# MrSwordFish/rvel-mcmc

Measured on AMD Instinct MI355X. Metric: walker-logL evals/sec (2-planet, 100 obs, 4096 walkers); ESS/sec, higher is better.
Workload: dtype f64

## Files before the change

include/rvmcmc.h:

```cpp
#ifndef RVMCMC_H
#define RVMCMC_H

#include <stddef.h>
#include <stdint.h>

#ifdef __cplusplus
extern "C" {
#endif

#define RVM_ABI_VERSION 12

#define RVM_STATUS_OK 0
#define RVM_STATUS_PRIOR 1
#define RVM_STATUS_ENCOUNTER 2
#define RVM_STATUS_NONFINITE 3
#define RVM_STATUS_UNRESOLVED 4
#define RVM_STATUS_SKIPPED 5

#define RVM_MAX_PLANETS 4
#define RVM_MAX_LEVELS 6
#define RVM_MAX_EPOCHS_PER_DIRECTION 1700
#define RVM_SMALA_MAX_PARAMS 20
#define RVM_RESOLVE_MAX_LIMIT 12

typedef struct {
    int32_t n_planets;
    double dt;
    int32_t n_levels;
    double npoints_norm;
    int32_t level_mult[RVM_MAX_LEVELS];
    double period_hint;
    int32_t inclined;
    double resolve_tol;
    int32_t resolve_max;
} rvm_config;

typedef struct rvm_plan rvm_plan;

int rvm_plan_create(const rvm_config* cfg, const double* t, const double* rv, const double* sigma, int32_t n_obs,
                    int32_t max_walkers, rvm_plan** out);
void rvm_plan_destroy(rvm_plan* plan);
int rvm_plan_info(const rvm_plan* plan, int32_t* steps_fwd, int32_t* steps_bwd, int32_t* epochs_fwd,
                  int32_t* epochs_bwd);
#define RVM_EXT_MAX_BYTES (4ull << 30)
int rvm_plan_extension(const rvm_plan* plan, int32_t* ext_mult);
int rvm_plan_set_verify_eccentricity(rvm_plan* plan, double e);

int rvm_plan_set_certain_reject(rvm_plan* plan, int32_t on);

int rvm_plan_faults(rvm_plan* plan, int32_t reset, int64_t* handoff_timeouts, int64_t* nonfinite,
                    int64_t* unresolved, int64_t* refined, int64_t* truncated, void* stream);
#define RVM_N_COUNTERS 7
int rvm_plan_counters(rvm_plan* plan, int32_t reset, int64_t* out, int32_t n, void* stream);
int rvm_plan_hedge_stats(rvm_plan* plan, int32_t reset, int64_t* hedged, int64_t* replayed, int64_t* missed,
                         void* stream);
int rvm_plan_hedge_marks(rvm_plan* plan, int32_t reset, int64_t* marked, int64_t* gave_up, void* stream);
int rvm_plan_hedge_waits(rvm_plan* plan, int32_t reset, int64_t* waited, int64_t* late_hits, int64_t* gave_way,
                         void* stream);
int rvm_plan_time_kernels(rvm_plan* plan, int32_t max_launches);
int rvm_plan_kernel_times(rvm_plan* plan, float* logl_ms, float* refine_ms, int32_t max, int32_t* n_out);
int rvm_plan_set_handoff_timeout(rvm_plan* plan, double seconds);

int rvm_logl_batch(const rvm_plan* plan, int32_t n_walkers, const double* params, double hill_factor,
                   double* logl_out, int32_t* status_out, double* rv_out, void* stream);


int rvm_stretch_propose(int32_t n_params, int32_t n_s0, int64_t s0_begin, const double* x, int32_t n_s1,
                        const double* c, double a, uint64_t seed, uint64_t iteration, uint32_t half,
                        const double* draws, double* q_out, double* z_out, void* stream);
int rvm_stretch_accept(int32_t n_params, int32_t n_s0, int64_t s0_begin, double* x, double* lnp, const double* q,
                       const double* lnp_new, const double* z, uint64_t seed, uint64_t iteration, uint32_t half,
                       const double* draws, int32_t* accepted, void* stream);

#define RVM_MAX_PARAM_ROWS (7 * RVM_MAX_PLANETS)
typedef struct rvm_param_map {
    int32_t n_rows;
    int32_t src[RVM_MAX_PARAM_ROWS];
    double base[RVM_MAX_PARAM_ROWS];
} rvm_param_map;

int rvm_stretch_half_step(const rvm_plan* plan, const rvm_param_map* map, int32_t n_params, int32_t n_s0,
                          int64_t s0_begin, double* x, double* x_aos, double* lnp, int32_t n_s1, const double* c_aos,
                          double a, uint64_t seed, uint64_t iteration, uint32_t half, double hill_factor,
                          double* lnp_new_out, int32_t* status_out, int32_t* accepted, void* stream);

int rvm_stretch_iteration_begin(const rvm_plan* plan, const rvm_param_map* map, int32_t n_params, int32_t n_loc,
                                int64_t s0_begin, int64_t s1_begin, double* x0, double* lnp0, const double* x1,
                                const double* lnp1, int32_t n_half, const double* c0, const double* c1, double a,
                                uint64_t seed, uint64_t iteration, double hill_factor, double* lnp_spec,
                                int32_t* status_spec, int32_t* dec, int32_t* accepted0, void* stream);
int rvm_stretch_iteration_end(int32_t n_params, int32_t n_loc, int64_t s0_begin, int64_t s1_begin, const double* x0,
                              double* x0_aos, const int32_t* dec, const int32_t* dec_all, double* x1, double* x1_aos,
                              double* lnp1, int32_t n_half, const double* c0, const double* c1,
                              const double* lnp_spec, const int32_t* status_spec, double a, uint64_t seed,
                              uint64_t iteration, int32_t* accepted1, double* lnp_new_out, int32_t* status_new_out,
                              void* stream);

int rvm_pt_stretch_propose(int32_t n_params, int32_t n_temps, int32_t n_half, const double* x, const double* c,
                           double a, uint64_t seed, uint64_t iteration, uint32_t half, const double* draws,
                           double* q_out, double* z_out, void* stream);
int rvm_pt_stretch_accept(int32_t n_params, int32_t n_temps, int32_t n_half, const double* betas, double* x,
                          double* lnp, const double* q, const double* lnp_new, const double* z, uint64_t seed,
                          uint64_t iteration, uint32_t half, const double* draws, int32_t* accepted, void* stream);
int rvm_pt_swap(int32_t n_params, int32_t n_temps, int32_t n_half, const double* betas, double* x0, double* x1,
                double* lnp0, double* lnp1, uint64_t seed, uint64_t iteration, const double* draws,
                int32_t* swapped, void* stream);

int rvm_pt_ladder_update(int32_t n_temps, int32_t n_half, const int32_t* swapped, const double* lnp0,
                         const double* lnp1, double kappa, double* betas, int64_t* swap_totals_prev,
                         double* ratios_out, int64_t* n_refused, double* lnp_moments, void* workspace,
                         void* stream);

int rvm_mh_propose(int32_t n_params, int32_t n_chains, int64_t chain_begin, const double* x, const double* scales,
                   double step_size, uint64_t seed, uint64_t iteration, const double* draws, double* q_out,
                   void* stream);
int rvm_mh_accept(int32_t n_params, int32_t n_chains, int64_t chain_begin, double* x, double* lnp, const double* q,
                  const double* lnp_new, uint64_t seed, uint64_t iteration, const double* draws, int32_t* accepted,
                  void* stream);
int rvm_mh_step(const rvm_plan* plan, const rvm_param_map* map, int32_t n_params, int32_t n_chains,
                int64_t chain_begin, double* x, double* lnp, const double* scales, double step_size, uint64_t seed,
                uint64_t iteration, double hill_factor, double* lnp_new_out, int32_t* status_out, int32_t* accepted,
                void* stream);

int rvm_fd_params(int32_t n_params, int32_t n_chains, const double* x, double rel_step, const double* floor_,
                  double* out, void* stream);

typedef struct {
    double* lp;
    double* grad;
    double* mu;
    double* L;
    double* G;
    double* logdet;
    int32_t* ok;
} rvm_smala_cache;

int rvm_smala_derive(int32_t n_params, int32_t n_chains, int32_t n_obs, const double* x, double rel_step,
                     const double* floor_, const double* lp_stencil, const int32_t* status_stencil,
                     const double* rv_stencil, const double* inv_sigma2, double npoints_norm, double alpha,
                     double eps, const rvm_smala_cache* out, void* stream);
int rvm_smala_metric(int32_t n_params, int32_t n_chains, const double* x, const double* lp, const int32_t* status,
// ... 55 lines not shown
```

rvel-mcmc_amd/csrc/host_sanitize.cpp:

```cpp
#include <algorithm>
#include <cmath>
#include <cstdio>
#include <cstdlib>
#include <cstring>
#include <vector>

#include "rvm_plan_host.h"

static int fails = 0;
static void expect(bool ok, const char* what) {
    if (!ok) {
        std::fprintf(stderr, "FAIL %s\n", what);
        fails++;
    }
}

static double exact_weight(const int* m, int k0, int n, int k) {
    long long num = 1, den = 1;
    for (int j = k0; j < n; j++) {
        if (j == k) continue;
        num *= (long long)m[k] * m[k];
        den *= (long long)m[k] * m[k] - (long long)m[j] * m[j];
    }
    return (double)num / (double)den;
}

static bool close_rel(double a, double b, double rel) { return std::fabs(a - b) <= rel * std::fabs(b); }

static double ulp_of(double x) { return std::nextafter(std::fabs(x), INFINITY) - std::fabs(x); }

struct Range {
    size_t off, bytes;
    bool wide;
};
static void check_block(const std::vector<Range>& r, size_t block_bytes, const char* what) {
    size_t end = 0;
    for (const Range& x : r) {
        expect(x.off >= end, what);
        expect(!x.wide || x.off % 8 == 0, what);
        end = x.off + x.bytes;
    }
    expect(end <= block_bytes, what);
}

static const char* const kKnobNames[] = {
    "RVM_SKIP_VARIANTS", "RVM_LATE_SPO",   "RVM_NO_LEVEL_SPLIT", "RVM_REFINE_TEAMS", "RVM_EAGER_SPLIT",
    "RVM_NO_EXTENSION",  "RVM_REFINE_SPLIT", "RVM_TEAMS_HINT",   "RVM_EAGER",        "RVM_EAGER_PASSES",
    "RVM_HEDGE",         "RVM_HEDGE_GROUPS", "RVM_HEDGE_MARK",   "RVM_HEDGE_WAIT",
    "RVM_LS_F0"};

static rvm::PlanKnobs knobs_with(const char* name, const char* value) {
    setenv(name, value, 1);
    const rvm::PlanKnobs K = rvm::read_plan_knobs();
    unsetenv(name);
    return K;
}

static void check_plan_host(const rvm_config& cfg, const std::vector<double>& t, const std::vector<double>& rv,
                            const std::vector<double>& sg) {
    using namespace rvm;
    const int n_obs = (int)t.size();
    for (const char* name : kKnobNames) unsetenv(name);
    const PlanKnobs K = read_plan_knobs();
    expect(K.skip_variants == 1 && K.late_spo == 96.0 && !K.no_level_split && K.n_teams == RVM_TEAMS_DEFAULT &&
               K.eager_split == 1 && !K.no_extension && K.refine_split && K.teams_hint && K.eager &&
               K.eager_passes == 1 && K.hedge_groups == RVM_HEDGE_GROUPS_MAX && K.hedge_mark == 1 &&
               K.hedge_wait == 1,
           "knob defaults");
    expect(knobs_with("RVM_REFINE_TEAMS", "9").n_teams == RVM_TEAMS_MAX, "RVM_REFINE_TEAMS=9 clamps");
    expect(knobs_with("RVM_HEDGE", "0").hedge_groups == 0, "RVM_HEDGE=0");
    expect(knobs_with("RVM_HEDGE_GROUPS", "3").hedge_groups == 3, "RVM_HEDGE_GROUPS=3");
    expect(knobs_with("RVM_EAGER_PASSES", "2").eager_passes == 2, "RVM_EAGER_PASSES=2");
    expect(knobs_with("RVM_SKIP_VARIANTS", "0").skip_variants == 0, "RVM_SKIP_VARIANTS=0");
    expect(knobs_with("RVM_HEDGE_WAIT", "0").hedge_wait == 0 && knobs_with("RVM_HEDGE_WAIT", "1").hedge_wait == 1 &&
               knobs_with("RVM_HEDGE_WAIT", "2").hedge_wait == 2 && knobs_with("RVM_HEDGE_WAIT", "x").hedge_wait == 1,
           "RVM_HEDGE_WAIT");

    int mult[RVM_MAX_LEVELS] = {}, max_mult = 0;
    expect(check_plan_config(&cfg, t.data(), rv.data(), sg.data(), n_obs, 4096, mult, &max_mult) == nullptr,
           "config ok");
    expect(mult[0] == 4 && mult[1] == 5 && mult[2] == 6 && mult[3] == 7 && max_mult == 7, "explicit ladder");
    {
        rvm_config h = cfg;
        h.n_levels = 3;
        std::memset(h.level_mult, 0, sizeof(h.level_mult));
        int hm[RVM_MAX_LEVELS] = {}, hmax = 0;
        expect(check_plan_config(&h, t.data(), rv.data(), sg.data(), n_obs, 64, hm, &hmax) == nullptr && hm[0] == 1 &&
                   hm[1] == 2 && hm[2] == 3 && hmax == 3,
               "harmonic ladder");
    }

    HostDir dir[2];
    expect(build_schedule(&cfg, mult, max_mult, t.data(), rv.data(), sg.data(), n_obs, dir) == nullptr, "schedule ok");
    std::vector<int> seen(n_obs, 0);
    int n_dup = 0;
    for (int d = 0; d < 2; d++) {
        const HostDir& D = dir[d];
        const size_t n = D.idx.size();
        expect(D.seg_n.size() == n && D.seg_len.size() == n && D.orv.size() == n && D.os2.size() == n,
               "schedule sizes");
        long long sum = 0, pre0 = 0, pre1 = 0;
        double tprev = 0.0;
        for (size_t i = 0; i < n; i++) {
            const int o = D.idx[i];
            expect(o >= 0 && o < n_obs && (d == 0) == (t[o] >= 0.0), "obs_idx direction");
            if (o >= 0 && o < n_obs) seen[o]++;
            const double at = std::fabs(t[o]), len = (d == 0 ? 1.0 : -1.0) * (at - tprev);
            expect(at >= tprev, "|t| non-decreasing");
            if (at == tprev) {
                n_dup += i > 0;
                expect(D.seg_n[i] == 0 && D.seg_len[i] == 0.0, "duplicate epoch: empty segment");
            } else {
                expect(D.seg_n[i] >= 1 && std::fabs(D.seg_len[i]) <= cfg.dt * (1.0 + 1e-9), "segment step <= dt");
                expect(std::fabs(D.seg_n[i] * D.seg_len[i] - len) <= 4.0 * ulp_of(len), "segment steps x step = length");
            }
            tprev = at;
            if ((int)i < D.split0) pre0 += D.seg_n[i];
            if ((int)i < D.split1) pre1 += D.seg_n[i];
            sum += D.seg_n[i];
        }
        expect(sum == D.total_steps, "sum(seg_n) = n_steps");
        expect(D.split0 >= 0 && D.split0 <= (int)n && D.split1 >= 0 && D.split1 <= (int)n, "split range");
        expect(pre0 == D.pre0 && pre1 == D.pre1, "pre = steps before the split");
    }
    expect(std::all_of(seen.begin(), seen.end(), [](int c) { return c == 1; }), "obs_idx is a permutation");
    expect(n_dup == 1, "one duplicate epoch");

    const size_t nf = dir[0].idx.size(), nb = dir[1].idx.size();
    rvm_config ad = cfg;
    ad.resolve_tol = 5e-7;
    ad.resolve_max = 6;
    DevPlan P{};
    fill_plan_scalars(&ad, mult, n_obs, nf, nb, 256, K, &P);
    expect(P.ext_mult == 0 && plan_wants_extension(P, K), "extension wanted, not yet applied");
    fill_plan_extension(&P);
    const int m5[5] = {4, 5, 6, 7, 8};
    for (int k = 0; k < 4; k++) expect(close_rel(P.lw[k], exact_weight(m5, 0, 4, k), 1e-14), "lw");
    for (int k = 1; k < 4; k++) expect(close_rel(P.lw3[k], exact_weight(m5, 1, 4, k), 1e-14), "lw3");
    for (int k = 0; k < 5; k++) expect(close_rel(P.lw5[k], exact_weight(m5, 0, 5, k), 1e-14), "lw5");
    expect(P.lw3[0] == 0.0 && P.lw[4] == 0.0 && P.lw[5] == 0.0 && P.lw5[5] == 0.0, "unused weights are zero");

    expect(P.fin_level == 3, "fin_level");
    expect(P.ext_mult == 8 && P.mult[4] == 8 && P.inv_ext == 0.125 && P.inv_mult[4] == 0.125, "ext_mult");
    expect(P.rmax == 6 && P.rtol_dir == 2.5e-7 && P.cut == 1 && P.n_teams == RVM_TEAMS_DEFAULT, "adaptive scalars");
    expect(P.hedge_wait_ticks == hedge_wait_bound(P.spin_ticks) && P.hedge_wait_ticks < (P.spin_ticks << 1),
           "hedge_wait_ticks");
    for (unsigned long long sp : {1ull, 2ull, 3ull, 4ull, 1000ull, 200000000ull, 1ull << 40, 1ull << 62})
        expect(hedge_wait_bound(sp) < sp && hedge_wait_bound(sp) < (sp << 1), "hedge_wait_bound");
    for (int k = 0; k < 4; k++) {
        const double nh = 2.0 * M_PI * cfg.dt / (mult[k] * cfg.period_hint), zn = 2.0 * nh * nh;
        expect(P.nt[k] == (zn <= 0.1 ? 6 : (zn <= 0.3 ? 7 : 8)) && P.spec[k] == (zn <= 0.04 ? 1 : 0), "nt / spec");
        expect(P.inv_mult[k] == 1.0 / mult[k], "inv_mult");
    }
    expect(P.ext_nt == P.nt[3] && P.ext_spec == P.spec[3] && P.nt[4] == P.nt[3] && P.spec[4] == P.spec[3],
           "ext nt / spec");
    expect(P.late_mult == (int)std::ceil(96 * 0.65 / 5.2 - 1e-9) && P.late_mult == 12, "late_mult");
    expect(P.lc_ring >= 2 && P.lc_ring <= RVM_LC_RING, "lc_ring range");
    expect((size_t)(cfg.n_levels + 1) * 32 * 8 * P.lc_ring <= RVM_LC_RING_BYTES, "lc_ring bytes");
    {
        DevPlan Q{};
        fill_plan_scalars(&cfg, mult, n_obs, nf, nb, 256, K, &Q);
        expect(Q.rmax == 0 && !plan_wants_extension(Q, K) && Q.ext_mult == 0, "no extension without resolve_tol");
        ad.resolve_max = 0;
        fill_plan_scalars(&ad, mult, n_obs, nf, nb, 256, K, &Q);
        expect(!plan_wants_extension(Q, K) && Q.ext_mult == 0, "no extension with resolve_max 0");
        expect(!plan_wants_extension(P, knobs_with("RVM_NO_EXTENSION", "1")), "RVM_NO_EXTENSION=1");
        fill_plan_scalars(&cfg, mult, n_obs, nf, nb, 256, knobs_with("RVM_LATE_SPO", "0"), &Q);
        expect(Q.late_mult == 0, "RVM_LATE_SPO=0");
    }

    for (int32_t mw : {1, 64, 6144}) {
        const size_t w = (size_t)mw, em = std::max(nf, nb);
        const DmemLayout D = dmem_layout(nf, nb, mw);
        check_block({{D.seg_h1[0], 8 * nf, true}, {D.obs_rv[0], 8 * nf, true}, {D.obs_s2[0], 8 * nf, true},
                     {D.seg_h1[1], 8 * nb, true}, {D.obs_rv[1], 8 * nb, true}, {D.obs_s2[1], 8 * nb, true},
                     {D.slots, 8 * w, true}, {D.counters, 8 * RVM_N_COUNTERS, true}, {D.seg_n[0], 4 * nf, false},
                     {D.obs_idx[0], 4 * nf, false}, {D.seg_n[1], 4 * nb, false}, {D.obs_idx[1], 4 * nb, false}},
                    D.bytes, "dmem layout");
        const LvLayout V = lv_layout(nf, nb, mw);
        expect(V.emax == (int32_t)em, "lv emax");
        check_block({{V.rv, 8 * 2 * em * w, true}, {V.enc, 4 * 2 * w, false}}, V.bytes, "lvmem layout");
        for (int teams : {1, 2, 4}) {
            const size_t nt = (size_t)std::max(teams, 2), xg = (w + 15) / 16 + 1;
            const XLayout X = x_layout(nf, nb, mw, teams);
            check_block({{X.lvx, 16 * em * w, true}, {X.rvp, 16 * em * w, true},
                         {X.rvp2, 16 * em * w * (teams - 1), true}},
                        X.bytes, "xmem layout");
            const RqLayout R = rq_layout(mw, teams);
            expect(R.xgroups == (int32_t)xg, "rq xgroups");
            check_block({{R.x, xg * nt * 256 * 8, true}, {R.xf, xg * nt * 2 * 8, true},
                         {R.t, xg * (nt - 1) * 1024 * 8, true}, {R.tf, xg * nt * 8, true}, {R.tb, xg * 8, true},
                         {R.c, 16 * w, true},
                         {R.w, 12 * w, false}, {R.n, 16, false}, {R.gen, 8, true}, {R.mark, 4 * w, false},
                         {R.depth, 8 * (RVM_DEPTH_WINDOW + 1), true}},
                        R.bytes, "rqmem layout");
            expect(R.tb == R.tf + xg * nt * 8, "rq_tb right behind rq_tf");
            expect(R.gen == R.n + 32 && R.mark == R.n + 64 && R.mark % 64 == R.n % 64, "rq_n | gen_dev | rq_mark");
        }
        const HLayout H = h_layout((int32_t)em, mw);
        const size_t hs = RVM_HEDGE_STRIDE;
        check_block({{H.hrv, 16 * em * hs, true}, {H.hsum, 48 * hs, true}, {H.hslot, 16 * hs, true},
                     {H.htab, 8 * w, true}, {H.hw, 8 * RVM_HW_WORDS, true}},
                    H.bytes, "hmem layout");
        expect(RVM_HW_STATS + 5 <= RVM_HW_MARK && RVM_HW_MARK + 2 * RVM_HEDGE_GROUPS_MAX <= RVM_HW_WAIT &&
                   RVM_HW_WAIT + 3 <= RVM_HW_WORDS,
               "hw words");
        const ELayout E = e_layout((int32_t)em, mw);
        check_block({{E.rve, 32 * em * w, true}, {E.esum, 96 * w, true},
                     {E.eflag, 8 * (RVM_EFLAG_WORDS * (size_t)((RVM_EAGER_MAX + 15) / 16) + 8), true}},
                    E.bytes, "emem layout");
    }
}

int main() {
    expect(rvm_abi_version() == RVM_ABI_VERSION, "abi version");
    rvm_config cfg{};
    cfg.n_planets = 2;
    cfg.dt = 0.65;
    cfg.n_levels = 4;
    cfg.npoints_norm = 100.0;
    const int mult[4] = {4, 5, 6, 7};
    std::memcpy(cfg.level_mult, mult, sizeof(mult));
    cfg.period_hint = 5.2;
    std::vector<double> t, rv, sg;
    for (int i = 0; i < 101; i++) {
        t.push_back(i % 2 ? -0.6 * i : 0.55 * (100 - i));
        rv.push_back(1e-4 * std::sin(i));
        sg.push_back(1.5e-4);
    }
    t[7] = t[9];
    rvm_plan* plan = nullptr;
    const int rc = rvm_plan_create(&cfg, t.data(), rv.data(), sg.data(), (int)t.size(), 4096, &plan);
    expect(rc == 0 || (rc < 0 && plan == nullptr), "plan_create valid input");
    if (rc == 0) rvm_plan_destroy(plan);
    check_plan_host(cfg, t, rv, sg);
    rvm_config bad = cfg;
    bad.n_levels = 0;
    expect(rvm_plan_create(&bad, t.data(), rv.data(), sg.data(), (int)t.size(), 64, &plan) < 0, "n_levels 0");
    bad = cfg;
    bad.level_mult[1] = 4;
    expect(rvm_plan_create(&bad, t.data(), rv.data(), sg.data(), (int)t.size(), 64, &plan) < 0, "dup multipliers");
    bad = cfg;
    bad.dt = -1.0;
    expect(rvm_plan_create(&bad, t.data(), rv.data(), sg.data(), (int)t.size(), 64, &plan) < 0, "negative dt");
    std::vector<double> tn = t;
    tn[3] = NAN;
    expect(rvm_plan_create(&cfg, tn.data(), rv.data(), sg.data(), (int)t.size(), 64, &plan) < 0, "nan epoch");
    expect(std::strlen(rvm_last_error()) > 0, "last_error");
    expect(rvm_logl_batch(nullptr, 1, nullptr, 1.0, nullptr, nullptr, nullptr, nullptr) < 0, "logl null plan");
    int64_t mk = -1, gu = -1;
    expect(rvm_plan_hedge_marks(nullptr, 0, &mk, &gu, nullptr) < 0 && mk == -1 && gu == -1, "hedge_marks null plan");
    int64_t lh = -1;
    expect(rvm_plan_hedge_waits(nullptr, 0, &mk, &lh, &gu, nullptr) < 0 && mk == -1 && lh == -1 && gu == -1,
           "hedge_waits null plan");
    rvm_param_map pm{};
    expect(rvm_stretch_half_step(nullptr, &pm, 10, 1, 0, nullptr, nullptr, nullptr, 1, nullptr, 2.0, 0, 0, 0, 1.0,
                                 nullptr, nullptr, nullptr, nullptr) < 0,
           "half_step null plan");
    expect(rvm_stretch_propose(0, 1, 0, nullptr, 1, nullptr, 2.0, 0, 0, 0, nullptr, nullptr, nullptr, nullptr) < 0,
           "propose bad");
    double d1 = 0.5;
    int32_t i1 = 0;
    expect(rvm_pt_stretch_propose(10, 0, 1, &d1, &d1, 2.0, 0, 0, 0, nullptr, &d1, &d1, nullptr) < 0, "pt n_temps 0");
    expect(rvm_pt_stretch_propose(10, 2, 1, &d1, &d1, 1.0, 0, 0, 0, nullptr, &d1, &d1, nullptr) < 0, "pt a = 1");
    expect(rvm_pt_stretch_propose(10, 1 << 16, 1 << 16, &d1, &d1, 2.0, 0, 0, 0, nullptr, &d1, &d1, nullptr) < 0,
           "pt int32 overflow");
    expect(rvm_pt_stretch_accept(10, 2, 1, nullptr, &d1, &d1, &d1, &d1, &d1, 0, 0, 0, nullptr, &i1, nullptr) < 0,
           "pt null betas");
    expect(rvm_pt_stretch_accept(10, 2, 1, &d1, &d1, &d1, &d1, &d1, &d1, 0, 0, 2, nullptr, &i1, nullptr) < 0,
           "pt half 2");
    expect(rvm_pt_swap(10, 2, 0, &d1, &d1, &d1, &d1, &d1, 0, 0, nullptr, &i1, nullptr) < 0, "pt n_half 0");
    expect(rvm_pt_swap(10, 1 << 15, 1 << 15, &d1, &d1, &d1, &d1, &d1, 0, 0, nullptr, &i1, nullptr) < 0,
           "pt swap int32 overflow");
    expect(rvm_pt_swap(10, 1, 4, nullptr, nullptr, nullptr, nullptr, nullptr, 0, 0, nullptr, nullptr, nullptr) == 0,
           "pt swap of one temperature");
    int64_t l1 = 0;
    expect(rvm_pt_ladder_update(3, 1, &i1, &d1, &d1, -1.0, &d1, &l1, &d1, &l1, nullptr, &d1, nullptr) < 0,
           "pt ladder kappa < 0");
    expect(rvm_pt_ladder_update(3, 1, &i1, &d1, &d1, 0.5, &d1, &l1, &d1, &l1, nullptr, nullptr, nullptr) < 0,
           "pt ladder null workspace");
    expect(rvm_pt_ladder_update(1 << 16, 1 << 15, &i1, &d1, &d1, 0.5, &d1, &l1, &d1, &l1, nullptr, &d1, nullptr) < 0,
           "pt ladder int32 overflow");
    expect(rvm_pt_ladder_update(1, 4, nullptr, nullptr, nullptr, 0.5, nullptr, nullptr, nullptr, nullptr, nullptr,
                                nullptr, nullptr) == 0,
           "pt ladder of one temperature");
    expect(rvm_chain_record(2, 4, &d1, 16, 0, INT64_MAX, &d1, 8, 0, nullptr, nullptr, nullptr) < 0,
           "chain record stride overflow");
    expect(rvm_chain_record(2, 4, &d1, 16, 0, 1, &d1, INT64_MAX, INT64_MAX - 1, nullptr, nullptr, nullptr) < 0,
           "chain record dst_col0 overflow");
    expect(rvm_chain_record(2, 4, &d1, 16, 0, 1, &d1, 8, 0, &d1, nullptr, nullptr) < 0, "chain record lone lnp_src");
    expect(rvm_chain_moments(&d1, 2, 4, 5, 5, &d1, &d1, nullptr) < 0, "chain moments empty range");
    expect(rvm_chain_autocov(&d1, &d1, 2, 4, 0, 10, INT32_MAX, 1 << 30, &d1, &d1, nullptr) < 0,
           "chain autocov lag overflow");
    expect(rvm_chain_autocov(&d1, &d1, 65534, 4, 0, INT64_MAX, 0, 1 << 30, &d1, &d1, nullptr) < 0,
           "chain autocov n_params * n_lags");
    expect(rvm_chain_autocov_workspace_bytes(10, 200, 17) == (size_t)8 * 10 * 32, "chain autocov workspace");
    expect(rvm_chain_autocov_workspace_bytes(1, 65535 * 256, 1 << 30) == (size_t)8 * ((size_t)1 << 30) * 65535,
           "chain autocov workspace, largest");
    expect(rvm_chain_autocov_workspace_bytes(65534, 4, 1 << 30) == 0, "chain autocov workspace, refused");
    expect(rvm_mh_accept(0, 1, 0, nullptr, nullptr, nullptr, nullptr, 0, 0, nullptr, nullptr, nullptr) < 0, "mh bad");
    expect(rvm_fd_params(10, 1, nullptr, 1e-6, nullptr, nullptr, nullptr) < 0, "fd bad");
    const int32_t rows[2] = {0, 0};
    expect(rvm_logl_derivs(nullptr, 1, nullptr, 2, rows, 1.0, nullptr, nullptr, nullptr, nullptr, nullptr, nullptr) < 0,
           "derivs null plan");
    expect(rvm_logl_derivs_workspace_bytes(256, 10) == (size_t)256 * 55 * 2 * 36, "derivs workspace");
    rvm_smala_cache c{};
    expect(rvm_smala_metric(10, 1, nullptr, nullptr, nullptr, nullptr, nullptr, 1.0, 0.5, &c, nullptr) < 0, "metric bad");
    std::printf("host sanitize driver: %d failures\n", fails);
    return fails;
}
```

rvel-mcmc_amd/csrc/rvm_internal.h:

```cpp
#pragma once
#include <stdint.h>

#include "../../include/rvmcmc.h"

namespace rvm {

constexpr int RVM_LS_RING = 64;
constexpr int RVM_LC_RING = 16;
constexpr int RVM_LC_RING_BYTES = 24 * 1024;
constexpr int RVM_LDS_PER_CU = 160 * 1024;
constexpr int RVM_INIT_DOUBLES = 8 * 64;
constexpr double RVM_EXT_ACCEPT = 1.0;
constexpr double RVM_CUT_EST_FACTOR = 100.0;
constexpr double RVM_FLOOR_BOUND = 4.0;
constexpr double RVM_CUT_ECC_FACTOR = 0.6712;
constexpr double RVM_CUT_GUARD_K = 10.0;
constexpr int RVM_CX_MIN_WALKERS = 32;
constexpr int RVM_EAGER_MAX = 512;
constexpr int RVM_EAGER_MIN = 32;
constexpr int RVM_EFLAG_WORDS = 8;
constexpr int RVM_TEAMS_MAX = 4;
constexpr int RVM_TEAMS_DEFAULT = 4;
constexpr int RVM_DEPTH_WINDOW = 8;
constexpr int RVM_HEDGE_GROUPS_MAX = 8;
constexpr int RVM_HEDGE_STRIDE = 512;
constexpr int RVM_HEDGE_CAND = RVM_HEDGE_STRIDE + 64;
constexpr int RVM_HEDGE_MAX_W = 12288;
constexpr int RVM_HW_STATS = 2 + 2 * RVM_HEDGE_GROUPS_MAX;
constexpr int RVM_HW_MARK = RVM_HW_STATS + 3 + 3;
constexpr int RVM_HW_WAIT = RVM_HW_MARK + 2 * RVM_HEDGE_GROUPS_MAX;
constexpr int RVM_HW_WORDS = RVM_HW_WAIT + 3;

struct DirSched {
    int32_t n_epochs;
    int32_t n_steps;
    int32_t split0, pre0, split1, pre1;
    const int32_t* seg_n;
    const double* seg_h1;
    const double* obs_rv;
    const double* obs_s2;
    const int32_t* obs_idx;
};

struct DevPlan {
    int32_t n_planets;
    int32_t n_levels;
    int32_t mult[RVM_MAX_LEVELS];
    int32_t nt[RVM_MAX_LEVELS];
    int32_t spec[RVM_MAX_LEVELS];
    int32_t late_mult;
    int32_t lc_ring;
    double inv_mult[RVM_MAX_LEVELS];
    double lw[RVM_MAX_LEVELS];
    double lw3[RVM_MAX_LEVELS];
    double rtol_dir;
    int32_t rmax;
    int32_t fin_level;
    int32_t cut;
    int32_t ext_mult, ext_nt, ext_spec;
    double inv_ext;
    double lw5[RVM_MAX_LEVELS + 1];
    double* lvx;
    double* rvp;
    double e2_guard;
    double e2_cut;
    double cut_guard_k;
    int32_t lvx_emax, lvx_stride;
    int32_t* rq_n;
    int32_t* rq_w;
    double* rq_c;
    int32_t rq_cap;
    uint32_t hedge_wait_ticks;
    int32_t* rq_mark;
    int32_t skip_variants;
    unsigned long long* rq_x;
    unsigned long long* rq_xf;
    int32_t rq_xgroups;
    unsigned long long* rq_t;
    unsigned long long* rq_tf;
    double* rvp2;
    int32_t n_teams;
    unsigned long long* depth_w;
    double* rve;
    double* esum;
    unsigned long long* eflag;
    int32_t eager_max;
    int32_t eager_passes;
    int32_t eager_split;
    int32_t hedge_groups;
    int32_t hedge_mark;
    int32_t hedge_wait;
    double* hrv;
    double* hsum;
    unsigned long long* hslot;
    unsigned long long* htab;
    unsigned long long* hw;
    unsigned long long* gen_dev;
    unsigned long long* counters;
    unsigned long long spin_ticks;
    double npoints;
    int32_t n_obs;
    int32_t inclined;
    int32_t n_cu;
    double* lv_rv;
    int32_t* lv_enc;
    int32_t lv_emax, lv_stride;
    DirSched fwd, bwd;
};

struct StretchArgs {
    const double* c;
    double* x;
    double* x_aos;
    double* lnp;
    int32_t* accepted;
    int64_t s0_begin;
    uint64_t seed, iteration;
    double a;
    int32_t n1, dim;
    uint32_t half;
    int32_t xstride;
    int32_t n_spec;
    const double* c0;
    const double* x1;
    int64_t s1_begin;
    int32_t* dec;
    const double* lnp1;
    const double* mh_scale;
    double mh_step;
    const double* fd_x;
    const double* fd_floor;
    double fd_rel;
    int32_t fd_n;
    int32_t src[RVM_MAX_PARAM_ROWS];
    double base[RVM_MAX_PARAM_ROWS];
};

struct IterEndArgs {
    int32_t dim, n, n_half;
    int64_t s0_begin, s1_begin;
    const double* x0;
    double* x0_aos;
    const int32_t* dec_local;
    const int32_t* dec_all;
    double* x1;
    double* x1_aos;
    double* lnp1;
    const double* c0;
    const double* c1;
    const double* lnp_spec;
    const int32_t* st_spec;
    double a;
    uint64_t seed, iteration;
    int32_t* accepted1;
    double* lnp_new_out;
    int32_t* status_new_out;
};

struct PtLadderArgs {
    int32_t T, Wh;
    const int32_t* swapped;
    const double* lnp0;
    const double* lnp1;
    double kappa;
    double* betas;
    int64_t* totals_prev;
    double* ratios;
    int64_t* n_refused;
    double* moments;
    int64_t* ws_totals;
    double* ws_moments;
};

struct SmalaCache {
    double* lp;
    double* grad;
    double* mu;
    double* L;
    double* G;
    double* logdet;
    int32_t* ok;
};

}
```

rvel-mcmc_amd/csrc/rvm_logl.hip:

```cpp
#include <hip/hip_runtime.h>
#include <math.h>

#include <algorithm>

#pragma clang fp contract(on)

#include "rvm_launch.h"
#include "rvm_walker.h"

#ifndef RVM_MAIN_G5
#define RVM_MAIN_G5 0
#endif

namespace rvm {

#ifdef RVM_PROFILE
#define RVM_PROF_SLOTS 18
#define RVM_PROF_MAX_WAVES 4096
__device__ unsigned long long rvm_prof[RVM_PROF_MAX_WAVES * RVM_PROF_SLOTS];
#define PROF_T(v) const unsigned long long v = __builtin_readcyclecounter()
#define PROF_COUNT(var) (var)++
#else
#define PROF_T(v)
#define PROF_COUNT(var)
// ... 396 lines not shown
                __builtin_amdgcn_s_setprio(1);
            if (lvl == hl) {
                if (pl_idx == 0 && valid) {
                    unsigned long long bits = (unsigned long long)__double_as_longlong(v0);
                    if (bits == RVM_LV_EMPTY) bits = 0x7FF8000000000000ULL;
                    __hip_atomic_store(lv1p, bits, __ATOMIC_RELAXED, __HIP_MEMORY_SCOPE_AGENT);
                }
                lv1p += P.lv_stride;
            } else {
                if (E > RING && !wfault) {
                    int seen = -1;
                    for (;;) {
                        const int cp = __builtin_amdgcn_readfirstlane(
                            __hip_atomic_load(s_cprog + ul, __ATOMIC_ACQUIRE, __HIP_MEMORY_SCOPE_WORKGROUP));
                        if (e - cp < RING) break;
                        if (cp != seen) {
                            seen = cp;
                            clk.restart();
                        } else if (clk.expired(P.spin_ticks)) {
                            wfault = true;
                            break;
                        }
                        __builtin_amdgcn_s_sleep(4);
                    }
                }
                if (pl_idx == 0) ring[((ul * NK + ks) * RING + rslot) * WPB + slot] = v0;
                if (lane == 0) __hip_atomic_store(&s_lvp[ul][ks], e + 1, __ATOMIC_RELEASE, __HIP_MEMORY_SCOPE_WORKGROUP);
                rslot = rslot + 1 == RING ? 0 : rslot + 1;
            }
        } else {
            if (lc_pair) {
                rem -= ns * wcost;
                if (lane == 0) __hip_atomic_store(s_rem + wv, rem, __ATOMIC_RELAXED, __HIP_MEMORY_SCOPE_WORKGROUP);
                const int ro = __builtin_amdgcn_readfirstlane(rem_oth), rm = __builtin_amdgcn_readfirstlane(rem);
                if (__builtin_amdgcn_readfirstlane((int)(ro < rm)))
                    __builtin_amdgcn_s_setprio(2);
                else
                    __builtin_amdgcn_s_setprio(1);
            }
            if (lvl == 0) {
                while (!wfault && e - next_c >= RC) {
                    lc_wait(next_c);
                    if (!wfault) lc_combine(next_c++);
                }
            } else if (E > RC && !wfault && e >= RC) {
                int seen = -1;
                for (;;) {
                    const int cp = __builtin_amdgcn_readfirstlane(
                        __hip_atomic_load(&s_lcc[grp], __ATOMIC_ACQUIRE, __HIP_MEMORY_SCOPE_WORKGROUP));
                    if (e - cp < RC) break;
                    if (cp != seen) {
                        seen = cp;
                        clk.restart();
                    } else if (clk.expired(P.spin_ticks)) {
                        wfault = true;
                        break;
                    }
                    __builtin_amdgcn_s_sleep(4);
                }
            }
            if (pl_idx == 0) lring[((size_t)(e % RC) * (nl + 1) + lvl) * WPB + slot] = v0;
            if (lane == 0) __hip_atomic_store(&s_lcp[grp][lvl], e + 1, __ATOMIC_RELEASE, __HIP_MEMORY_SCOPE_WORKGROUP);
            if (lvl == 0 && !wfault) {
                const int mn = min(lc_min(), e + 1);
                while (next_c < mn) lc_combine(next_c++);
            }
        }
        n1 = n1_next;
        len = len_next;
#ifdef RVM_PROFILE
        PROF_T(tc);
        t_seg += tb - ta;
        t_epo += tc - tb;
#endif
    }
    if (!dec && lvl == 0) {
        while (!wfault && next_c < E_int) {
            lc_wait(next_c);
            if (!wfault) lc_combine(next_c++);
        }
    }
    const int encflag = (int)(((s.encm >> lane) & kick_enc_bits<NP>()) != 0) |
                        (status == RVM_STATUS_PRIOR ? 2 : 0) | (wfault ? RVM_ENC_FAULT : 0);
    auto finish = [&](const int wo, const double chi2w, const int enc, const bool open, const double lbw, auto&& row,
                      const double z, const double u3, const double lnp0) __attribute__((always_inline)) {
        const int st = dir_status(enc, open, chi2w);
        const unsigned long long mine =
            st != RVM_STATUS_OK ? slot_status(st)
                                : (unsigned long long)__double_as_longlong(open ? -lbw : chi2w);
        const unsigned long long old =
            __hip_atomic_exchange(slots + wo, mine, __ATOMIC_RELAXED, __HIP_MEMORY_SCOPE_AGENT);
        if (old == RVM_SLOT_EMPTY) return;
        __hip_atomic_store(slots + wo, RVM_SLOT_EMPTY, __ATOMIC_RELAXED, __HIP_MEMORY_SCOPE_AGENT);
        int st_o = RVM_STATUS_OK;
        bool open_o = false;
        double v_o = 0.0;
        if (slot_is_status(old)) {
            st_o = (int)(old & 0xFF);
        } else {
            v_o = __longlong_as_double((long long)old);
            open_o = signbit(v_o);
            v_o = fabs(v_o);
        }
        const double v_m = open ? lbw : chi2w;
        const int sf = d == 0 ? st : st_o, sb = d == 0 ? st_o : st;
        const bool of = d == 0 ? open : open_o, ob = d == 0 ? open_o : open;
        const double cf = d == 0 ? v_m : v_o, cb = d == 0 ? v_o : v_m;
        int stw = sf != RVM_STATUS_OK ? sf : sb;
        if (stw == RVM_STATUS_UNRESOLVED && (sf == RVM_STATUS_ENCOUNTER || sb == RVM_STATUS_ENCOUNTER))
            stw = RVM_STATUS_ENCOUNTER;
        const double lp0 = -((cb + cf) / P.npoints);
        if (stw == RVM_STATUS_OK && (of || ob)) {
            int dmode = 0;
            double dz, du, dl;
            if (P.ext_mult > 0 && P.cut) accept_inputs(sa, wo, dmode, dz, du, dl);
            if (dmode != 0 && isfinite(lp0) && !accepts_at(sa, dmode, dz, du, dl, lp0)) {
                __hip_atomic_fetch_add(P.counters + 4, (unsigned long long)((of ? 1 : 0) + (ob ? 1 : 0)),
                                       __ATOMIC_RELAXED, __HIP_MEMORY_SCOPE_AGENT);
            } else {
                const int li = of && ob ? 0 : (of ? 1 : 2);
                const int ix = __hip_atomic_fetch_add(P.rq_n + li, 1, __ATOMIC_RELAXED, __HIP_MEMORY_SCOPE_AGENT);
                if (ix < P.rq_cap) {
                    P.rq_w[(size_t)li * P.rq_cap + ix] = wo;
                    P.rq_mark[wo] = (int32_t)__hip_atomic_load(P.gen_dev, __ATOMIC_RELAXED, __HIP_MEMORY_SCOPE_AGENT);
                    P.rq_c[wo] = of ? 0.0 : cf;
                    P.rq_c[(size_t)P.rq_cap + wo] = ob ? 0.0 : cb;
                    return;
                }
                stw = RVM_STATUS_NONFINITE;
            }
        }
        if (stw == RVM_STATUS_OK && !isfinite(lp0)) stw = RVM_STATUS_NONFINITE;
        walker_out<R>(P, sa, wo, stw, stw == RVM_STATUS_OK ? lp0 : -INFINITY, logl_out, status_out, row, z, u3, lnp0);
    };
    auto finish_recompute = [&](const int w_in, const double chi2w, const int enc, const bool open, const double lbw) __attribute__((always_inline)) {
        if (stretch) {
            int wo = w_in, k2, wk2, j2, jp2;
            double z2, zp2;
            asm volatile("" : "+v"(wo));
            stretch_slot(sa, wo, k2, wk2, z2, j2, zp2, jp2);
            auto row = [&](int r) { return walker_param(true, params, W, wk2, sa, r, z2, j2, k2, zp2, jp2); };
            finish(wo, chi2w, enc, open, lbw, row, z2,
                   stretch_u3(sa.seed, (uint64_t)(sa.s0_begin + wo), sa.iteration, sa.half), k2 == 0 ? sa.lnp[wo] : 0.0);
        } else if (mh) {
            auto row = [&](int r) { return walker_param(true, params, W, w_in, sa, r, 0.0, 0, 0, 0.0, 0); };
            finish(w_in, chi2w, enc, open, lbw, row, 0.0, mh_u(sa.seed, (uint64_t)(sa.s0_begin + w_in), sa.iteration),
                   sa.lnp[w_in]);
        } else {
            auto row = [&](int) { return 0.0; };
            finish(w_in, chi2w, enc, open, lbw, row, 0.0, 0.0, 0.0);
        }
    };

    int dummy_redo = 0;
    auto extend_pass = [&](const int gr, const int dr, const uint64_t need_m, bool& need, double& chi2w, int& enc,
                           double& c5o, double& ddo) __attribute__((always_inline)) {
        const DirSched& SR = dr ? P.bwd : P.fwd;
        const int Er = SR.n_epochs;
        const double* r_dir = dec ? s_sched + (size_t)dr * 4 * emax2 : l_dir;
        const double* r_len = r_dir;
        const double* r_rv = r_dir + Er;
        const double* r_s2 = r_dir + 2 * Er;
        const int* r_n = reinterpret_cast<const int*>(r_dir + 3 * Er);
        const int* r_idx = r_n + Er;
        {
            const double* in = l_init + (size_t)gr * RVM_INIT_DOUBLES + lane;
            s.rx = in[0];
            s.ry = in[64];
            s.vx = in[128];
            s.vy = in[192];
            s.rz = in[256];
            s.vz = in[320];
            s.r = in[384];
            s.ir = in[448];
            s.encm = 0;
        }
        KickPrep<NP> kq{};
        if (Er > 0) kq = kick_prep<NP, L, D3>(s, 1.875);
        const int mx = P.ext_mult;
        const int ntx = P.ext_nt;
        const double ix = P.inv_ext;
        const int cs = lane & (WPB - 1);
        const bool cl = lane < WPB && ((need_m >> lane) & 1);
        const int wo = w0 + cs;
        const size_t xb = (size_t)dr * P.lvx_emax * P.lvx_stride + (cl ? wo : 0);
        const double* xs = P.lvx + xb;
        const double* xr = P.rvp + xb;
        double a5 = cl && Er > 0 ? xs[0] : 0.0, a4 = cl && Er > 0 ? xr[0] : 0.0;
        double c5 = 0.0, dd = 0.0;
        int x_off = 0, x_bo = 4;
        for (int e = 0; e < Er; e++) {
            const bool nx = cl && e + 1 < Er;
            const double b5 = nx ? xs[(size_t)(e + 1) * P.lvx_stride] : 0.0;
            const double b4 = nx ? xr[(size_t)(e + 1) * P.lvx_stride] : 0.0;
            const int ns = r_n[e] * mx;
            if (ns > 0) {
                const double h = r_len[e] * ix;
                if (P.ext_spec && ntx <= 6) {
                    if (x_off == 0) {
                        if (segment<6, true, D3, NP, L, RVM_MAIN_G5 != 0>(s, kq, h, ns, dummy_redo)) {
                            x_off = x_bo;
                            x_bo = x_bo < 64 ? 2 * x_bo : 64;
                        } else {
                            x_bo = 4;
                        }
                    } else {
                        segment<6, false, D3, NP, L, RVM_MAIN_G5 != 0>(s, kq, h, ns, dummy_redo);
                        x_off--;
                    }
                } else if (ntx <= 6)
                    segment<6, false, D3, NP, L, RVM_MAIN_G5 != 0>(s, kq, h, ns, dummy_redo);
                else if (ntx == 7)
                    segment<7, false, D3, NP, L, RVM_MAIN_G5 != 0>(s, kq, h, ns, dummy_redo);
                else
                    segment<8, false, D3, NP, L, RVM_MAIN_G5 != 0>(s, kq, h, ns, dummy_redo);
            }
            const double v = star_vx<NP, L>(s);
            const double vx = __shfl(v, cs * L);
            if (cl) {
                const double r = a4;
                const double r5 = a5 + P.lw5[nl] * vx;
                const double q = r5 - r_rv[e];
                c5 += (q * q) / r_s2[e];
                dd += fabs((r5 - r) * (q + (r - r_rv[e]))) / r_s2[e];
                if (rv_out != nullptr && wo < W) rv_out[(size_t)r_idx[e] * W + wo] = r5;
            }
            a5 = b5;
            a4 = b4;
        }
        const bool xenc = ((s.encm >> (cs * L)) & kick_enc_bits<NP>()) != 0;
        if (cl) {
            c5o = c5;
            ddo = dd;
// ... 286 lines not shown
                encc = (s_encl[ul][1][slot] | s_encl[ul][2][slot]) & 1;
                enc = s_encl[ul][0][slot] | ((s_encl[ul][1][slot] | s_encl[ul][2][slot]) & ~1);
            }
            {
                f1 = valid ? f1 : 0;
                if (ballot(f1 < 0) != 0 && !hung) {
                    do {
                        __builtin_amdgcn_s_sleep(2);
                        hung = clk.expired(P.spin_ticks);
                        f1 = valid ? __hip_atomic_load(e1p, __ATOMIC_RELAXED, __HIP_MEMORY_SCOPE_AGENT) : 0;
                    } while (ballot(f1 < 0) != 0 && !hung);
                }
                if (valid && pl_idx == 0) __hip_atomic_store(e1p, -1, __ATOMIC_RELAXED, __HIP_MEMORY_SCOPE_AGENT);
                const int f1p = f1 > 0 ? f1 : 0;
                if (P.rtol_dir < INFINITY) {
                    enc |= f1p & ~1;
                    encc |= f1p & 1;
                } else {
                    enc |= f1p;
                }
            }
            const bool cenc = encc != 0 && (enc & 1) == 0;
            if (hung) {
                chi2w = __builtin_nan("");
                enc |= RVM_ENC_FAULT;
                if (!dirty && lane == 0)
                    __hip_atomic_fetch_add(P.counters, 1ull, __ATOMIC_RELAXED, __HIP_MEMORY_SCOPE_AGENT);
            }
#ifdef RVM_PROFILE
            const unsigned long long rt_arr = __builtin_amdgcn_s_memrealtime();
#endif
            bool need = P.rtol_dir < INFINITY && valid && pl_idx == 0 && enc == 0 &&
                        (est / P.npoints > P.rtol_dir || !isfinite(chi2w) || !isfinite(est) ||
                         (P.ext_mult > 0 && e2w > P.e2_guard) || cenc);
            if (cenc && need && !lsx && P.ext_mult > 0)
                for (int e = 0; e < E; e++) P.rvp[(size_t)(d * P.lvx_emax + e) * P.lvx_stride + w] = __builtin_nan("");
            if (need && P.rmax == 0) {
                enc |= RVM_ENC_UNRESOLVED;
                need = false;
            }
            const bool need0 = need;
            const double chi2m = chi2w;
            if (lsx) {
                const uint64_t nx = ballot(need);
                if (lane == 0 && nx)
                    __hip_atomic_fetch_add(P.counters + 3, (unsigned long long)__builtin_popcountll(nx),
                                           __ATOMIC_RELAXED, __HIP_MEMORY_SCOPE_AGENT);
                if (need) {
                    if (s_encl[ul][3][slot] & 1) {
                        enc |= 1;
                        chi2w = c5x;
                        need = false;
                    } else if (!cenc && ddx <= RVM_EXT_ACCEPT * P.rtol_dir * P.npoints) {
                        chi2w = c5x;
                        need = false;
                    }
                }
            }
            if (!lsx && P.ext_mult > 0 && ballot(need) != 0) {
                if (valid && pl_idx == 0) {
                    s_fchi[ul][slot] = chi2w;
                    s_fenc[ul][slot] = enc | (need ? 16 : 0) | (cenc ? 32 : 0) | (e2w > P.e2_cut ? 64 : 0);
                    s_fx[0][ul][slot] = est;
                }
                __builtin_amdgcn_fence(__ATOMIC_RELEASE, "wavefront");
                __builtin_amdgcn_wave_barrier();
                const bool cl = lane < WPB && w0 + lane < W;
                double c2 = cl ? s_fchi[ul][lane] : 0.0;
                const int f = cl ? s_fenc[ul][lane] : 0;
                const double es = cl ? s_fx[0][ul][lane] : 0.0;
                const double cm = c2;
                int en = f & 15;
                bool nd = (f & 16) != 0;
                const bool cn = (f & 32) != 0;
                const uint64_t nm = ballot(nd);
                if (lane == 0)
                    __hip_atomic_fetch_add(P.counters + 3, (unsigned long long)__builtin_popcountll(nm),
                                           __ATOMIC_RELAXED, __HIP_MEMORY_SCOPE_AGENT);
                double xc5 = 0.0, xdd = 0.0;
                extend_pass(ul, d, nm, nd, c2, en, xc5, xdd);
                const double lb = cn ? 0.0 : direction_lb(nd, cm, es, (f & 16) != 0 && ((f & 64) == 0 || P.cut_guard_k > 0.0), xc5,
                                                                 (f & 64) != 0 ? P.cut_guard_k * xdd : xdd);
                if (cl) finish_recompute(w0 + lane, c2, en, nd, lb);
            } else if (valid && pl_idx == 0) {
                if (lsx && need) {
                    const double* rg = ring + (size_t)(ul * 4 + 2) * RING * WPB + slot;
                    for (int e = 0; e < E; e++)
                        P.rvp[(size_t)(d * P.lvx_emax + e) * P.lvx_stride + w] = cenc ? __builtin_nan("") : rg[(size_t)e * WPB];
                }
                finish_recompute(w, chi2w, enc, need,
                                 cenc ? 0.0 : direction_lb(need, chi2m, est, lsx && need0 && (e2w <= P.e2_cut || P.cut_guard_k > 0.0), c5x,
                                                          e2w <= P.e2_cut ? ddx : P.cut_guard_k * ddx));
            }
#ifdef RVM_PROFILE
            prof_dec(rt_arr, nl - 1);
#endif
        }
        return;
    }
#ifdef RVM_PROFILE
    PROF_T(t_end);
    const int gw = (blockIdx.y * gridDim.x + blockIdx.x) * (blockDim.x >> 6) + wv;
    if (lane == 0 && gw < RVM_PROF_MAX_WAVES) {
        unsigned long long* o = rvm_prof + (size_t)gw * RVM_PROF_SLOTS;
        o[0] = t_start;
        o[1] = t_pro;
        o[2] = t_seg;
        o[3] = t_epo;
        o[4] = t_end;
        o[5] = rt_start;
        o[6] = __builtin_amdgcn_s_memrealtime();
        o[7] = (unsigned long long)lvl | ((unsigned long long)blockIdx.y << 8) | ((unsigned long long)mult << 16);
        o[8] = (unsigned long long)redo;
        o[9] = (unsigned long long)E;
        o[10] = (unsigned long long)(unsigned)__builtin_amdgcn_s_getreg((31 << 11) | 4);
        o[14] = t_p1;
        o[15] = t_p2;
        o[16] = t_p3;
        o[17] = t_p4;
    }
#endif
}

template <int NPV, bool D3V, bool DECV>
static size_t lds_budget() {
    static size_t budget[64] = {};
    int dev = 0;
    if (hipGetDevice(&dev) != hipSuccess || dev < 0 || dev >= 64) {
        (void)hipGetLastError();
        return 32 * 1024;
    }
    if (budget[dev] == 0) {
        const void* f = reinterpret_cast<const void*>(&logl_kernel<NPV, D3V, DECV>);
        hipFuncAttributes fa{};
        size_t b = 32 * 1024;
        if (hipFuncGetAttributes(&fa, f) == hipSuccess && fa.sharedSizeBytes < (size_t)RVM_LDS_PER_CU) {
            const size_t lim = (size_t)RVM_LDS_PER_CU - fa.sharedSizeBytes;
            if (hipFuncSetAttribute(f, hipFuncAttributeMaxDynamicSharedMemorySize, (int)lim) == hipSuccess)
                b = lim;
            else if (fa.sharedSizeBytes < 64 * 1024)
                b = 64 * 1024 - fa.sharedSizeBytes;
        }
        (void)hipGetLastError();
        budget[dev] = b;
    }
    return budget[dev];
}

template <int NPV, bool D3V>
static hipError_t launch_logl_t(const DevPlan& P, int W, const double* params, double hill_factor,
                                unsigned long long* slots, double* logl, int32_t* status, double* rv_out,
                                const StretchArgs& sa, hipStream_t stream, int* dry_blocks) {
    const int lpw = LanesPerWalker<NPV>::value;
    const int wpb = 64 / lpw;
    const int groups = (W + wpb - 1) / wpb;
    static const bool pairs_env = [] {
        const char* e = getenv("RVM_CX_PAIRS");
        return !(e && e[0] == '0');
    }();
    const bool pairs = NPV == 3 && !D3V && pairs_env && P.ext_mult > 0 && rv_out == nullptr && P.n_cu > 0 &&
                       2 * groups > P.n_cu && groups <= P.n_cu && W >= RVM_CX_MIN_WALKERS;
    const int G = (!pairs && P.n_cu > 0 && 2 * groups > P.n_cu && 2 * P.n_levels * 64 <= 512) ? 2 : 1;
    dim3 grid((groups + G - 1) / G, 2);
    const bool cx = G == 1 && P.ext_mult > 0 && rv_out == nullptr && W >= RVM_CX_MIN_WALKERS;
    dim3 block(64 * (P.n_levels + (cx ? 1 : 0)) * G);
    const int emax = P.fwd.n_epochs > P.bwd.n_epochs ? P.fwd.n_epochs : P.bwd.n_epochs;
    const size_t rows = (size_t)(D3V ? 7 : 5) * NPV;
    const bool fused = sa.c != nullptr || sa.mh_scale != nullptr;
    const size_t init = P.rmax > 0 ? (size_t)RVM_INIT_DOUBLES * sizeof(double) : 0;
    const size_t lc_ring = (size_t)P.lc_ring * (P.n_levels + 1) * wpb * sizeof(double);
    size_t smem = (size_t)emax * 4 * sizeof(double) + (fused ? (rows + 3) * G * wpb * sizeof(double) : 0) + G * init +
                  G * lc_ring;
    int nA = 0, tB = 8, splitA = 0, lsx = 0;
    if (P.lv_rv != nullptr && W <= P.lv_stride && P.n_levels == 4 && P.n_cu > 0 && P.ext_mult > 0 &&
        rv_out == nullptr && G == 2 && emax <= RVM_LS_RING) {
        const int units = 2 * groups;
// ... 127 lines not shown
```

rvel-mcmc_amd/csrc/rvm_plan.hip:

```cpp
#include <algorithm>
#include <cmath>
#include <cstdlib>
#include <cstring>

#include "rvm_launch.h"
#include "rvm_plan.h"
#include "rvm_plan_host.h"

using rvm::fail;
using rvm::hip_fail;

namespace {

template <class T>
T* at(void* block, size_t offset) {
    return reinterpret_cast<T*>(reinterpret_cast<unsigned char*>(block) + offset);
}

template <class T>
const T* put(std::vector<unsigned char>& host, void* block, size_t offset, const std::vector<T>& v) {
    if (!v.empty()) std::memcpy(host.data() + offset, v.data(), v.size() * sizeof(T));
    return at<T>(block, offset);
}

// ... 15 lines not shown
    rvm::DirSched* S[2] = {&plan->dev.fwd, &plan->dev.bwd};
    for (int dd = 0; dd < 2; dd++) {
        const rvm::HostDir& D = dir[dd];
        S[dd]->n_epochs = (int32_t)D.idx.size();
        S[dd]->n_steps = plan->steps[dd] = (int32_t)D.total_steps;
        S[dd]->split0 = D.split0;
        S[dd]->pre0 = D.pre0;
        S[dd]->split1 = D.split1;
        S[dd]->pre1 = D.pre1;
        S[dd]->seg_h1 = put(host, plan->dmem, L.seg_h1[dd], D.seg_len);
        S[dd]->obs_rv = put(host, plan->dmem, L.obs_rv[dd], D.orv);
        S[dd]->obs_s2 = put(host, plan->dmem, L.obs_s2[dd], D.os2);
        S[dd]->seg_n = put(host, plan->dmem, L.seg_n[dd], D.seg_n);
        S[dd]->obs_idx = put(host, plan->dmem, L.obs_idx[dd], D.idx);
    }
    plan->slots = at<unsigned long long>(plan->dmem, L.slots);
    for (int32_t i = 0; i < max_walkers; i++)
        at<unsigned long long>(host.data(), L.slots)[i] = 0x7FF4DEADBEEF0001ULL;
    plan->dev.counters = at<unsigned long long>(plan->dmem, L.counters);
    plan->max_walkers = max_walkers;
    e = hipMemcpy(plan->dmem, host.data(), L.bytes, hipMemcpyHostToDevice);
    return e == hipSuccess ? 0 : hip_fail(e, "rvm_plan_create: hipMemcpy");
}

int device_cus() {
    int dev = 0, ncu = 0;
    if (hipGetDevice(&dev) != hipSuccess ||
        hipDeviceGetAttribute(&ncu, hipDeviceAttributeMultiprocessorCount, dev) != hipSuccess)
        ncu = 0;
    return ncu;
}

void alloc_level_split(rvm_plan* plan, size_t nf, size_t nb, const rvm::PlanKnobs& K) {
    rvm::DevPlan& P = plan->dev;
    if (!rvm::plan_wants_level_split(P, plan->max_walkers, K)) return;
    const rvm::LvLayout L = rvm::lv_layout(nf, nb, plan->max_walkers);
    if (!alloc_filled(&plan->lvmem, L.bytes, 0xFF)) return;
    P.lv_rv = at<double>(plan->lvmem, L.rv);
    P.lv_enc = at<int32_t>(plan->lvmem, L.enc);
    P.lv_emax = L.emax;
    P.lv_stride = plan->max_walkers;
    plan->lv_bytes = L.bytes;
}

void alloc_extension(rvm_plan* plan, size_t nf, size_t nb, const rvm::PlanKnobs& K) {
    rvm::DevPlan& P = plan->dev;
    if (!rvm::plan_wants_extension(P, K)) return;
    const rvm::XLayout L = rvm::x_layout(nf, nb, plan->max_walkers, K.n_teams);
    if (L.bytes > RVM_EXT_MAX_BYTES) return;
    if (hipMalloc(&plan->xmem, L.bytes) != hipSuccess) {
        plan->xmem = nullptr;
        (void)hipGetLastError();
        return;
    }
    rvm::fill_plan_extension(&P);
    P.lvx = at<double>(plan->xmem, L.lvx);
    P.rvp = at<double>(plan->xmem, L.rvp);
    P.rvp2 = K.n_teams >= 2 ? at<double>(plan->xmem, L.rvp2) : nullptr;
    P.lvx_emax = L.emax;
    P.lvx_stride = plan->max_walkers;
}

int alloc_work_lists(rvm_plan* plan, const rvm::PlanKnobs& K) {
    rvm::DevPlan& P = plan->dev;
    if (P.rmax <= 0) return 0;
    const rvm::RqLayout L = rvm::rq_layout(plan->max_walkers, K.n_teams);
    if (hipMalloc(&plan->rqmem, L.bytes) != hipSuccess || hipMemset(plan->rqmem, 0, L.bytes) != hipSuccess ||
        hipDeviceSynchronize() != hipSuccess) {
        (void)hipGetLastError();
        return fail(-3, "rvm_plan_create: hipMalloc of the refinement work lists failed");
    }
    P.rq_x = K.refine_split ? at<unsigned long long>(plan->rqmem, L.x) : nullptr;
    P.rq_xf = at<unsigned long long>(plan->rqmem, L.xf);
    P.rq_t = K.n_teams >= 2 ? at<unsigned long long>(plan->rqmem, L.t) : nullptr;
    P.rq_tf = at<unsigned long long>(plan->rqmem, L.tf);
    P.rq_c = at<double>(plan->rqmem, L.c);
    P.rq_w = at<int32_t>(plan->rqmem, L.w);
    P.rq_n = at<int32_t>(plan->rqmem, L.n);
    P.gen_dev = at<unsigned long long>(plan->rqmem, L.gen);
    P.rq_mark = at<int32_t>(plan->rqmem, L.mark);
    P.depth_w = K.teams_hint ? at<unsigned long long>(plan->rqmem, L.depth) : nullptr;
    P.rq_cap = plan->max_walkers;
    P.rq_xgroups = L.xgroups;
    const unsigned long long gen1 = 1;
    if (hipMemcpy(P.gen_dev, &gen1, sizeof(gen1), hipMemcpyHostToDevice) != hipSuccess) {
        (void)hipGetLastError();
        return fail(-3, "rvm_plan_create: initialising the launch generation failed");
    }
    return 0;
}

void side_drop(rvm_plan* plan) {
    (void)hipGetLastError();
    if (plan->ev_fork) (void)hipEventDestroy(plan->ev_fork);
    if (plan->ev_join) (void)hipEventDestroy(plan->ev_join);
    if (plan->side) (void)hipStreamDestroy(plan->side);
    plan->side = nullptr;
    plan->ev_fork = plan->ev_join = nullptr;
    plan->dev.hedge_groups = 0;
}

bool side_create(rvm_plan* plan) {
    if (hipStreamCreateWithFlags(&plan->side, hipStreamNonBlocking) == hipSuccess &&
        hipEventCreateWithFlags(&plan->ev_fork, hipEventDisableTiming) == hipSuccess &&
        hipEventCreateWithFlags(&plan->ev_join, hipEventDisableTiming) == hipSuccess)
        return true;
    side_drop(plan);
    return false;
}

void setup_side_features(rvm_plan* plan, const rvm::PlanKnobs& K) {
    rvm::DevPlan& P = plan->dev;
    const int32_t mw = plan->max_walkers;
    const bool refines = P.rmax >= 2 && P.rvp != nullptr && P.gen_dev != nullptr && P.n_levels <= 4 &&
                         mw >= rvm::RVM_EAGER_MIN;
    if (K.hedge_groups > 0 && refines && P.n_cu >= 4) {
        const rvm::HLayout L = rvm::h_layout(P.lvx_emax, mw);
        if (alloc_filled(&plan->hmem, L.bytes, 0)) {
            P.hrv = at<double>(plan->hmem, L.hrv);
            P.hsum = at<double>(plan->hmem, L.hsum);
            P.hslot = at<unsigned long long>(plan->hmem, L.hslot);
            P.htab = at<unsigned long long>(plan->hmem, L.htab);
            P.hw = at<unsigned long long>(plan->hmem, L.hw);
            P.hedge_groups = K.hedge_groups;
            P.hedge_mark = K.hedge_mark;
            P.hedge_wait = K.hedge_wait;
        }
    }
    if (!(refines && K.eager)) {
        if (P.hedge_groups > 0) (void)side_create(plan);
        return;
    }
    const rvm::ELayout L = rvm::e_layout(P.lvx_emax, P.lvx_stride);
    if (alloc_filled(&plan->emem, L.bytes, 0) && side_create(plan)) {
        P.rve = at<double>(plan->emem, L.rve);
        P.esum = at<double>(plan->emem, L.esum);
        P.eflag = at<unsigned long long>(plan->emem, L.eflag);
        P.eager_max = std::min<int>(mw, rvm::RVM_EAGER_MAX);
        P.eager_passes = K.eager_passes;
    } else {
        side_drop(plan);
        if (plan->emem) (void)hipFree(plan->emem);
        plan->emem = nullptr;
    }
}

int prepare_kernels(const rvm::DevPlan& P) {
    const hipError_t pe = rvm::prepare_logl(P);
    if (pe != hipSuccess)
        return fail(-1, pe == hipErrorInvalidConfiguration
                            ? "rvm_plan_create: the epoch schedule does not fit the likelihood kernel's LDS "
                              "(too many epochs in one direction)"
                            : "rvm_plan_create: n_planets has no kernel instantiation");
    if (rvm::prepare_refine(P) != hipSuccess)
        return fail(-1, "rvm_plan_create: the epoch schedule does not fit the refinement kernel's LDS "
                        "(too many epochs in one direction for the adaptive resolution)");
    return 0;
}

int read_hw_words(rvm_plan* plan, const char* who, int first, int n, int32_t reset, void* stream,
                  unsigned long long* h) {
    if (!plan) return fail(-1, std::string(who) + ": null plan");
    std::memset(h, 0, n * sizeof(*h));
    if (plan->dev.hw == nullptr) return 0;
    hipStream_t st = (hipStream_t)stream;
    unsigned long long* d = plan->dev.hw + first;
// ... 49 lines not shown
    if (plan->rqmem) (void)hipFree(plan->rqmem);
    if (plan->lvmem) (void)hipFree(plan->lvmem);
    if (plan->xmem) (void)hipFree(plan->xmem);
    if (plan->dmem) (void)hipFree(plan->dmem);
    delete plan;
}

int rvm_plan_set_certain_reject(rvm_plan* plan, int32_t on) {
    if (!plan) return fail(-1, "rvm_plan_set_certain_reject: null plan");
    plan->dev.cut = on ? 1 : 0;
    return 0;
}

int rvm_plan_set_verify_eccentricity(rvm_plan* plan, double e) {
    if (!plan) return fail(-1, "rvm_plan_set_verify_eccentricity: null plan");
    if (std::isnan(e) || e >= 1.0) return fail(-1, "rvm_plan_set_verify_eccentricity: e must be < 1 (<= 0: off)");
    plan->dev.e2_guard = e > 0.0 ? e * e : INFINITY;
    {
        const char* cf = getenv("RVM_CUT_FACTOR");
        const double ec = 1.0 - (1.0 - e) * (cf ? atof(cf) : rvm::RVM_CUT_ECC_FACTOR);
        const char* cg = getenv("RVM_CUT_GUARD");
        plan->dev.e2_cut = e > 0.0 && !(cg && atoi(cg) == 0) ? ec * ec : INFINITY;
        const char* ck = getenv("RVM_CUT_GUARD_K");
        plan->dev.cut_guard_k = ck ? atof(ck) : rvm::RVM_CUT_GUARD_K;
    }
    return 0;
}

int rvm_plan_extension(const rvm_plan* plan, int32_t* ext_mult) {
    if (!plan) return fail(-1, "rvm_plan_extension: null plan");
    if (ext_mult) *ext_mult = plan->dev.ext_mult;
    return 0;
}

int rvm_plan_counters(rvm_plan* plan, int32_t reset, int64_t* out, int32_t n, void* stream) {
    if (!plan) return fail(-1, "rvm_plan_counters: null plan");
    if (n < 0 || (n > 0 && !out)) return fail(-1, "rvm_plan_counters: bad output array");
    hipStream_t st = (hipStream_t)stream;
    unsigned long long h[RVM_N_COUNTERS] = {};
    hipError_t e = hipMemcpyAsync(h, plan->dev.counters, sizeof(h), hipMemcpyDeviceToHost, st);
    if (e == hipSuccess) e = hipStreamSynchronize(st);
    if (e != hipSuccess) return hip_fail(e, "rvm_plan_counters");
    for (int i = 0; i < n; i++) out[i] = i < RVM_N_COUNTERS ? (int64_t)h[i] : 0;
    if (reset) {
        if (plan->lvmem) e = hipMemsetAsync(plan->lvmem, 0xFF, plan->lv_bytes, st);
        if (e == hipSuccess) e = hipMemsetAsync(plan->dev.counters, 0, sizeof(h), st);
        if (e == hipSuccess) e = hipStreamSynchronize(st);
        if (e != hipSuccess) return hip_fail(e, "rvm_plan_counters: reset");
    }
    return 0;
}

int rvm_plan_hedge_stats(rvm_plan* plan, int32_t reset, int64_t* hedged, int64_t* replayed, int64_t* missed,
                         void* stream) {
    unsigned long long h[3];
    const int rc = read_hw_words(plan, "rvm_plan_hedge_stats", rvm::RVM_HW_STATS, 3, reset, stream, h);
    if (rc != 0) return rc;
    if (hedged) *hedged = (int64_t)h[0];
    if (replayed) *replayed = (int64_t)h[1];
    if (missed) *missed = (int64_t)h[2];
    return 0;
}

int rvm_plan_hedge_marks(rvm_plan* plan, int32_t reset, int64_t* marked, int64_t* gave_up, void* stream) {
    unsigned long long h[2];
    const int rc = read_hw_words(plan, "rvm_plan_hedge_marks", rvm::RVM_HW_STATS + 3, 2, reset, stream, h);
    if (rc != 0) return rc;
    if (marked) *marked = (int64_t)h[0];
    if (gave_up) *gave_up = (int64_t)h[1];
    return 0;
}

int rvm_plan_hedge_waits(rvm_plan* plan, int32_t reset, int64_t* waited, int64_t* late_hits, int64_t* gave_way,
                         void* stream) {
    unsigned long long h[3];
    const int rc = read_hw_words(plan, "rvm_plan_hedge_waits", rvm::RVM_HW_WAIT, 3, reset, stream, h);
    if (rc != 0) return rc;
    if (waited) *waited = (int64_t)h[0];
    if (late_hits) *late_hits = (int64_t)h[1];
    if (gave_way) *gave_way = (int64_t)h[2];
    return 0;
}

int rvm_plan_faults(rvm_plan* plan, int32_t reset, int64_t* handoff_timeouts, int64_t* nonfinite,
                    int64_t* unresolved, int64_t* refined, int64_t* truncated, void* stream) {
    if (!plan) return fail(-1, "rvm_plan_faults: null plan");
    int64_t c[RVM_N_COUNTERS] = {};
    const int rc = rvm_plan_counters(plan, reset, c, RVM_N_COUNTERS, stream);
    if (rc != 0) return rc;
    if (handoff_timeouts) *handoff_timeouts = c[0];
    if (nonfinite) *nonfinite = c[1];
    if (unresolved) *unresolved = c[2];
    if (refined) *refined = c[3];
    if (truncated) *truncated = c[4];
    return 0;
}

int rvm_plan_time_kernels(rvm_plan* plan, int32_t max_launches) {
    if (!plan) return fail(-1, "rvm_plan_time_kernels: null plan");
    if (max_launches < 0 || max_launches > 4096) return fail(-1, "rvm_plan_time_kernels: max_launches out of range");
    while ((int32_t)plan->tev.size() < 3 * max_launches) {
        hipEvent_t ev;
        const hipError_t e = hipEventCreate(&ev);
        if (e != hipSuccess) return hip_fail(e, "rvm_plan_time_kernels: hipEventCreate");
        plan->tev.push_back(ev);
    }
    plan->tcap = max_launches;
    plan->tn = 0;
    return 0;
}

int rvm_plan_kernel_times(rvm_plan* plan, float* logl_ms, float* refine_ms, int32_t max, int32_t* n_out) {
    if (!plan || max < 0) return fail(-1, "rvm_plan_kernel_times: bad arguments");
    const int n = std::min(plan->tn, max);
    for (int i = 0; i < n; i++) {
        hipError_t e = hipEventSynchronize(plan->tev[3 * i + 2]);
        float a = 0.0f, b = 0.0f;
        if (e == hipSuccess) e = hipEventElapsedTime(&a, plan->tev[3 * i], plan->tev[3 * i + 1]);
        if (e == hipSuccess) e = hipEventElapsedTime(&b, plan->tev[3 * i + 1], plan->tev[3 * i + 2]);
        if (e != hipSuccess) return hip_fail(e, "rvm_plan_kernel_times");
        if (logl_ms) logl_ms[i] = a;
        if (refine_ms) refine_ms[i] = b;
    }
    if (n_out) *n_out = n;
    plan->tn = 0;
    plan->tcap = 0;
    return 0;
}

int rvm_plan_set_handoff_timeout(rvm_plan* plan, double seconds) {
    if (!plan) return fail(-1, "rvm_plan_set_handoff_timeout: null plan");
    if (!(seconds > 0.0) || !(seconds < 1e9)) return fail(-1, "rvm_plan_set_handoff_timeout: seconds out of range");
    const double ticks = seconds * 1e8;
    plan->dev.spin_ticks = ticks < 1.0 ? 1ull : (unsigned long long)ticks;
    plan->dev.hedge_wait_ticks = rvm::hedge_wait_bound(plan->dev.spin_ticks);
    return 0;
}

int rvm_plan_info(const rvm_plan* plan, int32_t* sf, int32_t* sb, int32_t* ef, int32_t* eb) {
    if (!plan) return fail(-1, "rvm_plan_info: null plan");
    if (sf) *sf = plan->steps[0];
    if (sb) *sb = plan->steps[1];
    if (ef) *ef = plan->dev.fwd.n_epochs;
    if (eb) *eb = plan->dev.bwd.n_epochs;
    return 0;
}

}
```

rvel-mcmc_amd/csrc/rvm_plan_host.cpp:

```cpp
#include "rvm_plan_host.h"

#include <algorithm>
#include <cmath>
#include <cstdlib>

#ifndef RVM_EAGER_DEFAULT
#define RVM_EAGER_DEFAULT true
#endif
#ifndef RVM_EAGER_PASSES_DEFAULT
#define RVM_EAGER_PASSES_DEFAULT 1
#endif

namespace rvm {

static bool starts(const char* s, char c) { return s && s[0] == c; }

PlanKnobs read_plan_knobs() {
    PlanKnobs K;
    K.skip_variants = starts(getenv("RVM_SKIP_VARIANTS"), '0') ? 0 : 1;
    const char* ls = getenv("RVM_LATE_SPO");
    K.late_spo = ls ? atof(ls) : 96.0;
    K.no_level_split = false;
#ifdef RVM_PROFILE
    K.no_level_split = starts(getenv("RVM_NO_LEVEL_SPLIT"), '1');
#endif
    K.n_teams = RVM_TEAMS_DEFAULT;
    if (const char* tp = getenv("RVM_REFINE_TEAMS")) K.n_teams = std::max(1, std::min(atoi(tp), RVM_TEAMS_MAX));
    K.eager_split = starts(getenv("RVM_EAGER_SPLIT"), '0') ? 0 : 1;
    K.no_extension = starts(getenv("RVM_NO_EXTENSION"), '1');
    K.refine_split = !starts(getenv("RVM_REFINE_SPLIT"), '0');
    K.teams_hint = !starts(getenv("RVM_TEAMS_HINT"), '0');
    const char* eg = getenv("RVM_EAGER");
    K.eager = eg ? eg[0] == '1' : RVM_EAGER_DEFAULT;
    const char* ep = getenv("RVM_EAGER_PASSES");
    K.eager_passes = starts(ep, '1') ? 1 : (starts(ep, '2') ? 2 : RVM_EAGER_PASSES_DEFAULT);
    K.hedge_groups = starts(getenv("RVM_HEDGE"), '0') ? 0 : RVM_HEDGE_GROUPS_MAX;
    if (const char* hn = getenv("RVM_HEDGE_GROUPS"))
        K.hedge_groups = std::min(K.hedge_groups, std::max(0, std::min(atoi(hn), (int)RVM_HEDGE_GROUPS_MAX)));
    K.hedge_mark = starts(getenv("RVM_HEDGE_MARK"), '0') ? 0 : 1;
    const char* hwt = getenv("RVM_HEDGE_WAIT");
    K.hedge_wait = starts(hwt, '0') ? 0 : (starts(hwt, '2') ? 2 : 1);
    return K;
}

const char* check_plan_config(const rvm_config* cfg, const double* t, const double* rv, const double* sigma,
                              int32_t n_obs, int32_t max_walkers, int mult[RVM_MAX_LEVELS], int* max_mult) {
    if (cfg->n_planets < 1 || cfg->n_planets > RVM_MAX_PLANETS) return "rvm_plan_create: n_planets out of range";
    if (cfg->n_levels < 1 || cfg->n_levels > RVM_MAX_LEVELS) return "rvm_plan_create: n_levels out of range";
    if (!(cfg->dt > 0.0) || !std::isfinite(cfg->dt)) return "rvm_plan_create: dt must be > 0";
    if (n_obs < 0 || max_walkers < 1) return "rvm_plan_create: bad sizes";
    if (!(cfg->npoints_norm != 0.0)) return "rvm_plan_create: npoints_norm must be nonzero";
    bool harmonic = true;
    for (int k = 0; k < cfg->n_levels; k++) harmonic = harmonic && cfg->level_mult[k] == 0;
    *max_mult = 1;
    for (int k = 0; k < cfg->n_levels; k++) {
        mult[k] = harmonic ? k + 1 : cfg->level_mult[k];
        if (mult[k] < 1 || mult[k] > 64) return "rvm_plan_create: level_mult out of range (1..64)";
        for (int j = 0; j < k; j++)
            if (mult[j] == mult[k]) return "rvm_plan_create: level_mult entries must be distinct";
        *max_mult = std::max(*max_mult, mult[k]);
    }
    if (!(cfg->period_hint >= 0.0) || !std::isfinite(cfg->period_hint))
        return "rvm_plan_create: period_hint must be >= 0";
    if (std::isnan(cfg->resolve_tol) || cfg->resolve_max < 0 || cfg->resolve_max > RVM_RESOLVE_MAX_LIMIT)
        return "rvm_plan_create: resolve_tol must be a number and resolve_max in 0..12";
    for (int i = 0; i < n_obs; i++)
        if (!std::isfinite(t[i]) || !std::isfinite(rv[i]) || !std::isfinite(sigma[i]))
            return "rvm_plan_create: non-finite observation";
    return nullptr;
}

static void split_point(const HostDir& D, double frac, int32_t* split, int32_t* pre) {
    const double target = frac * (double)D.total_steps;
    long long cum = 0, best_cum = 0;
    int best = 0;
    double best_d = target;
    for (size_t i = 0; i < D.seg_n.size(); i++) {
        cum += D.seg_n[i];
        const double dist = std::fabs((double)cum - target);
        if (dist < best_d) {
            best_d = dist;
            best = (int)i + 1;
            best_cum = cum;
        }
    }
    *split = best;
    *pre = (int32_t)best_cum;
}

const char* build_schedule(const rvm_config* cfg, const int* mult, int max_mult, const double* t, const double* rv,
                           const double* sigma, int32_t n_obs, HostDir dir[2]) {
    const int rmax = cfg->resolve_tol > 0.0 ? cfg->resolve_max : 0;
    double f0 = 0.5;
    if (cfg->n_levels == 4) f0 = (double)(mult[3] + mult[0] - mult[2]) / (2.0 * mult[0]) + 0.11;
#ifdef RVM_PROFILE
    if (const char* ef = getenv("RVM_LS_F0")) f0 = atof(ef);
#endif
    f0 = std::min(1.0, std::max(0.0, f0));
    for (int dd = 0; dd < 2; dd++) {
        HostDir& D = dir[dd];
        for (int i = 0; i < n_obs; i++)
            if ((dd == 0) == (t[i] >= 0.0)) D.idx.push_back(i);
        std::stable_sort(D.idx.begin(), D.idx.end(), [&](int a, int b) { return std::fabs(t[a]) < std::fabs(t[b]); });
        const double sign = dd == 0 ? 1.0 : -1.0;
        double tprev = 0.0;
        for (int i : D.idx) {
            const double at = std::fabs(t[i]);
            const double len = at - tprev;
            tprev = at;
            int n = len > 0.0 ? (int)std::ceil(len / cfg->dt - 1e-9) : 0;
            if (len > 0.0 && n < 1) n = 1;
            D.seg_n.push_back(n);
            D.seg_len.push_back(n > 0 ? sign * len / n : 0.0);
            D.orv.push_back(rv[i]);
            D.os2.push_back(sigma[i] * sigma[i]);
            D.total_steps += n;
        }
        if ((D.total_steps * (long long)max_mult) << rmax > (1LL << 30))
            return "rvm_plan_create: dt too small for the epoch span";
        if (D.idx.size() > (size_t)RVM_MAX_EPOCHS_PER_DIRECTION)
            return "rvm_plan_create: too many epochs in one direction (the schedule is staged in LDS)";
        split_point(D, f0, &D.split0, &D.pre0);
        split_point(D, 0.5, &D.split1, &D.pre1);
    }
// ... 76 lines not shown
void fill_plan_extension(DevPlan* Pp) {
    DevPlan& P = *Pp;
    const int nl = P.n_levels, fin = P.fin_level;
    int m5[RVM_MAX_LEVELS + 1];
    for (int k = 0; k < nl; k++) m5[k] = P.mult[k];
    m5[nl] = P.mult[fin] + 1;
    lagrange_at_zero(m5, 0, nl + 1, P.lw5);
    P.ext_mult = m5[nl];
    P.ext_nt = P.nt[fin];
    P.ext_spec = P.spec[fin];
    P.inv_ext = 1.0 / m5[nl];
    P.mult[nl] = P.ext_mult;
    P.nt[nl] = P.ext_nt;
    P.spec[nl] = P.ext_spec;
    P.inv_mult[nl] = P.inv_ext;
}

bool plan_wants_level_split(const DevPlan& P, int32_t max_walkers, const PlanKnobs& K) {
    const int wpb = walkers_per_group(P.n_planets);
    const int64_t groups = ((int64_t)max_walkers + wpb - 1) / wpb;
    bool inc = P.n_levels == 4 && !K.no_level_split;
    for (int k = 1; inc && k < 4; k++) inc = P.mult[k] > P.mult[k - 1];
    return inc && P.n_cu > 0 && 2 * groups > P.n_cu;
}

static size_t take(size_t& end, size_t bytes) {
    end += bytes;
    return end - bytes;
}
static size_t epochs_max(size_t nf, size_t nb) { return std::max<size_t>(std::max(nf, nb), 1); }

DmemLayout dmem_layout(size_t nf, size_t nb, int32_t max_walkers) {
    DmemLayout L{};
    const size_t n[2] = {nf, nb};
    for (int d = 0; d < 2; d++) {
        L.seg_h1[d] = take(L.bytes, n[d] * sizeof(double));
        L.obs_rv[d] = take(L.bytes, n[d] * sizeof(double));
        L.obs_s2[d] = take(L.bytes, n[d] * sizeof(double));
    }
    L.slots = take(L.bytes, (size_t)max_walkers * sizeof(unsigned long long));
    L.counters = take(L.bytes, RVM_N_COUNTERS * sizeof(unsigned long long));
    for (int d = 0; d < 2; d++) {
        L.seg_n[d] = take(L.bytes, n[d] * sizeof(int32_t));
        L.obs_idx[d] = take(L.bytes, n[d] * sizeof(int32_t));
    }
    L.bytes += 64;
    return L;
}

LvLayout lv_layout(size_t nf, size_t nb, int32_t max_walkers) {
    LvLayout L{};
    L.emax = (int32_t)epochs_max(nf, nb);
    L.rv = take(L.bytes, (size_t)(2 * (int64_t)L.emax * max_walkers) * sizeof(double));
    L.enc = take(L.bytes, (size_t)(2 * (int64_t)max_walkers) * sizeof(int32_t));
    return L;
}

XLayout x_layout(size_t nf, size_t nb, int32_t max_walkers, int n_teams) {
    XLayout L{};
    L.emax = (int32_t)epochs_max(nf, nb);
    const size_t bl = 2 * (size_t)L.emax * (size_t)max_walkers * sizeof(double);
    L.lvx = take(L.bytes, bl);
    L.rvp = take(L.bytes, bl);
    L.rvp2 = take(L.bytes, ((size_t)n_teams - 1) * bl);
    return L;
}

RqLayout rq_layout(int32_t max_walkers, int n_teams) {
    RqLayout L{};
    const size_t xg = (size_t)(((int64_t)max_walkers + 15) / 16 + 1), nt = (size_t)std::max(n_teams, 2);
    const size_t u64 = sizeof(unsigned long long);
    L.xgroups = (int32_t)xg;
    L.x = take(L.bytes, xg * nt * 2 * 2 * 64 * u64);
    L.xf = take(L.bytes, xg * nt * 2 * u64);
    L.t = take(L.bytes, xg * (nt - 1) * 16 * 64 * u64);
    L.tf = take(L.bytes, xg * nt * u64);
    L.tb = take(L.bytes, xg * u64);
    L.c = take(L.bytes, 2 * (size_t)max_walkers * sizeof(double));
    L.w = take(L.bytes, (3 * (size_t)max_walkers * sizeof(int32_t) + 7) & ~(size_t)7);
    L.n = take(L.bytes, 64);
    L.gen = L.n + 32;
    L.mark = take(L.bytes, ((size_t)max_walkers * sizeof(int32_t) + 63) & ~(size_t)63);
    L.depth = take(L.bytes, (RVM_DEPTH_WINDOW + 1) * u64);
    return L;
}

HLayout h_layout(int32_t lvx_emax, int32_t max_walkers) {
    HLayout L{};
    const size_t hs = RVM_HEDGE_STRIDE, w = sizeof(double);
    L.hrv = take(L.bytes, 2 * (size_t)lvx_emax * hs * w);
    L.hsum = take(L.bytes, 6 * hs * w);
    L.hslot = take(L.bytes, 2 * hs * w);
    L.htab = take(L.bytes, (size_t)max_walkers * w);
    L.hw = take(L.bytes, RVM_HW_WORDS * w);
    return L;
}

ELayout e_layout(int32_t lvx_emax, int32_t lvx_stride) {
    ELayout L{};
    const size_t plane = (size_t)lvx_emax * lvx_stride;
    L.rve = take(L.bytes, 4 * plane * sizeof(double));
    L.esum = take(L.bytes, 12 * (size_t)lvx_stride * sizeof(double));
    L.eflag = take(L.bytes, (RVM_EFLAG_WORDS * (size_t)((RVM_EAGER_MAX + 15) / 16) + 8) * sizeof(double));
    return L;
}

}
```

rvel-mcmc_amd/csrc/rvm_plan_host.h:

```cpp
#pragma once
#include <cstddef>
#include <vector>

#include "rvm_internal.h"

namespace rvm {

struct PlanKnobs {
    int32_t skip_variants;
    double late_spo;
    bool no_level_split;
    int32_t n_teams;
    int32_t eager_split;
    bool no_extension;
    bool refine_split;
    bool teams_hint;
    bool eager;
    int32_t eager_passes;
    int32_t hedge_groups;
    int32_t hedge_mark;
    int32_t hedge_wait;
};
PlanKnobs read_plan_knobs();

const char* check_plan_config(const rvm_config* cfg, const double* t, const double* rv, const double* sigma,
                              int32_t n_obs, int32_t max_walkers, int mult[RVM_MAX_LEVELS], int* max_mult);

struct HostDir {
    std::vector<int32_t> idx, seg_n;
    std::vector<double> seg_len, orv, os2;
    long long total_steps = 0;
    int32_t split0 = 0, pre0 = 0, split1 = 0, pre1 = 0;
};
const char* build_schedule(const rvm_config* cfg, const int* mult, int max_mult, const double* t, const double* rv,
                           const double* sigma, int32_t n_obs, HostDir dir[2]);

void lagrange_at_zero(const int* m, int k0, int n, double* w);

inline int walkers_per_group(int n_planets) { return n_planets == 1 ? 64 : (n_planets == 2 ? 32 : 16); }

void fill_plan_scalars(const rvm_config* cfg, const int* mult, int32_t n_obs, size_t nf, size_t nb, int n_cu,
                       const PlanKnobs& K, DevPlan* P);
uint32_t hedge_wait_bound(unsigned long long spin_ticks);
bool plan_wants_extension(const DevPlan& P, const PlanKnobs& K);
void fill_plan_extension(DevPlan* P);
bool plan_wants_level_split(const DevPlan& P, int32_t max_walkers, const PlanKnobs& K);

struct DmemLayout {
    size_t seg_h1[2], obs_rv[2], obs_s2[2], slots, counters, seg_n[2], obs_idx[2], bytes;
};
DmemLayout dmem_layout(size_t nf, size_t nb, int32_t max_walkers);
struct LvLayout {
    size_t rv, enc, bytes;
    int32_t emax;
};
LvLayout lv_layout(size_t nf, size_t nb, int32_t max_walkers);
struct XLayout {
    size_t lvx, rvp, rvp2, bytes;
    int32_t emax;
};
XLayout x_layout(size_t nf, size_t nb, int32_t max_walkers, int n_teams);
struct RqLayout {
    size_t x, xf, t, tf, tb, c, w, n, gen, mark, depth, bytes;
    int32_t xgroups;
};
RqLayout rq_layout(int32_t max_walkers, int n_teams);
struct HLayout {
    size_t hrv, hsum, hslot, htab, hw, bytes;
};
HLayout h_layout(int32_t lvx_emax, int32_t max_walkers);
struct ELayout {
    size_t rve, esum, eflag, bytes;
};
ELayout e_layout(int32_t lvx_emax, int32_t lvx_stride);

}
```

rvel-mcmc_amd/csrc/rvm_refine_impl.h:

```cpp
#pragma once
#include <hip/hip_runtime.h>
#include <math.h>

#pragma clang fp contract(on)

#include "rvm_walker.h"

#ifndef RVM_REFINE_GUESS
#define RVM_REFINE_GUESS 0
#endif
#ifndef RVM_REFINE_RELAXED_COUNT
#define RVM_REFINE_RELAXED_COUNT 0
#endif

namespace rvm {

#ifdef RVM_PROFILE
#define RVM_RPROF_SLOTS 24
#define RVM_RPROF_MAX_WAVES 4096
static __device__ unsigned long long rvm_rprof[RVM_RPROF_MAX_WAVES * RVM_RPROF_SLOTS];
#define RPROF_T(v) const unsigned long long v = __builtin_readcyclecounter()
#define RPROF_RT(v) const unsigned long long v = __builtin_amdgcn_s_memrealtime()
#else
#define RPROF_T(v)
// ... 2 lines not shown

__device__ __forceinline__ bool claim_item(gu64* w, unsigned long long gen, unsigned long long code) {
    unsigned long long v = __hip_atomic_load(w, __ATOMIC_RELAXED, __HIP_MEMORY_SCOPE_AGENT);
    for (;;) {
        if ((v >> 8) == gen) return false;
        unsigned long long expect = v;
        if (__hip_atomic_compare_exchange_strong(w, &expect, (gen << 8) | code, __ATOMIC_RELAXED, __ATOMIC_RELAXED,
                                                 __HIP_MEMORY_SCOPE_AGENT))
            return true;
        v = expect;
    }
}

__device__ __forceinline__ void hedge_mark_unneeded(const int32_t* rq_w, const int rq_cap,
                                                    const unsigned long long* htab, unsigned long long* hw_,
                                                    const int n0, const int n1, const int n2,
                                                    const unsigned long long gen, const int hedge, const int wpb) {
    const int lane = threadIdx.x & 63;
    unsigned need = 0;
    for (int l2 = 0; l2 < 3; l2++) {
        int n = l2 == 0 ? n0 : (l2 == 1 ? n1 : n2);
        n = n < rq_cap ? n : rq_cap;
        for (int i = lane; i < n; i += 64) {
            const int wl = rq_w[(size_t)l2 * rq_cap + i];
            if (wl < 0 || wl >= rq_cap) continue;
            const unsigned long long tb = __hip_atomic_load((gu64*)htab + wl, __ATOMIC_RELAXED, __HIP_MEMORY_SCOPE_AGENT);
            const int hg = (int)(tb & 0xFFFF) / wpb;
            if ((tb >> 16) != gen || hg >= RVM_HEDGE_GROUPS_MAX) continue;
            if (l2 != 2) need |= 1u << (2 * hg);
            if (l2 != 1) need |= 1u << (2 * hg + 1);
        }
    }
    for (int d = 32; d >= 1; d >>= 1) need |= (unsigned)__shfl_xor((int)need, d, 64);
    gu64* hw = (gu64*)hw_;
    const bool mark = lane < hedge && lane < 2 * RVM_HEDGE_GROUPS_MAX && !((need >> lane) & 1u);
    if (mark) __hip_atomic_store(hw + RVM_HW_MARK + lane, (gen << 8) | 1ull, __ATOMIC_RELAXED, __HIP_MEMORY_SCOPE_AGENT);
    const unsigned long long nm = __builtin_popcountll(ballot(mark));
    if (lane == 0 && nm)
        __hip_atomic_fetch_add(hw + RVM_HW_STATS + 3, nm, __ATOMIC_RELAXED, __HIP_MEMORY_SCOPE_AGENT);
}

__device__ __forceinline__ int hedge_wait_poll(const DevPlan& P, const unsigned long long gen, const int wme,
                                               const bool o0, const bool o1, const int wpb, const gu64* tbw,
                                               const gu64* tdone) {
    const unsigned long long done = (gen << 8) | 2ull, stop = (gen << 8) | 3ull;
    auto state = [&](const int dd, const bool want) -> int {
        if (!want) return 0;
        const unsigned long long tb = __hip_atomic_load((gu64*)P.htab + wme, __ATOMIC_RELAXED, __HIP_MEMORY_SCOPE_AGENT);
        const int ix = (int)(tb & 0xFFFF);
        if ((tb >> 16) != gen || ix >= RVM_HEDGE_STRIDE || ix / wpb >= RVM_HEDGE_GROUPS_MAX) return 2;
        if (__hip_atomic_load((gu64*)P.hslot + (size_t)dd * RVM_HEDGE_STRIDE + ix, __ATOMIC_RELAXED,
                              __HIP_MEMORY_SCOPE_AGENT) != ((gen << 16) | (unsigned long long)wme))
            return 2;
        const unsigned long long w =
            __hip_atomic_load((gu64*)P.hw + 2 + 2 * (ix / wpb) + dd, __ATOMIC_RELAXED, __HIP_MEMORY_SCOPE_AGENT);
        return w == done ? 0 : (w == stop ? 2 : 1);
    };
    SpinClock clk;
    clk.restart();
    for (bool first = true;; first = false) {
        const int s0 = state(0, o0), s1 = state(1, o1);
        if (ballot(s0 == 2 || s1 == 2) != 0) return first ? -1 : 0;
        if (ballot(s0 == 1 || s1 == 1) == 0) return 1;
        const bool give = __hip_atomic_load(tbw, __ATOMIC_RELAXED, __HIP_MEMORY_SCOPE_AGENT) == ((gen << 8) | 1ull) ||
                          __hip_atomic_load(tdone, __ATOMIC_RELAXED, __HIP_MEMORY_SCOPE_AGENT) == done ||
                          clk.expired(P.hedge_wait_ticks);
        if (__builtin_amdgcn_readfirstlane((int)give)) return 0;
        __builtin_amdgcn_s_sleep(2);
    }
}

__device__ __forceinline__ unsigned long long pass_ticks(const DevPlan& P, int rf) {
    const unsigned long long t = P.spin_ticks << (rf < RVM_RESOLVE_MAX_LIMIT ? rf : RVM_RESOLVE_MAX_LIMIT);
    constexpr unsigned long long cap = 6000000000ull;
    return t < cap ? t : (P.spin_ticks > cap ? P.spin_ticks : cap);
}

struct DirState {
    int open;
    double chi, lb, pest, best, bchi;
};

constexpr int RVM_REFINE_HM = 5;
template <int NP, bool D3, int NW>
__global__ __launch_bounds__((NW == RVM_REFINE_HM ? 4 : NW) * 64) void refine_kernel(
    const DevPlan P, const int W, const double* __restrict__ params, const double hill_factor,
    double* __restrict__ rv_out, double* __restrict__ logl_out, int32_t* __restrict__ status_out, const StretchArgs sa,
    const int eager, const int hedge) {
    constexpr bool HM = NW == RVM_REFINE_HM;
    constexpr int L = LanesPerWalker<NP>::value;
    constexpr int WPB = 64 / L;
    constexpr int PR = D3 ? 7 : 5;
    constexpr int R = PR * NP;
    const int wv = threadIdx.x >> 6;
    const int lane = threadIdx.x & 63;
    const int slot = lane / L;
    const int pl_idx = lane % L;
    const int nl = P.n_levels;
    RPROF_T(pt_entry);
    RPROF_RT(prt_entry);
#ifdef RVM_PROFILE
    unsigned long long p_seg = 0, p_epo = 0, p_steps = 0, p_wait = 0, p_pass = 0;
    unsigned long long p_look = 0, p_info = 0, p_need = 0, p_barr = 0;
    int p_lvl = -1;
#endif

    __shared__ int s_n[3];
    __shared__ unsigned long long s_gen;
    __shared__ int s_depth;
    if (threadIdx.x == 0) {
        for (int i = 0; i < 3; i++) s_n[i] = __hip_atomic_load(P.rq_n + i, __ATOMIC_RELAXED, __HIP_MEMORY_SCOPE_AGENT);
        const unsigned long long g0 = __hip_atomic_load(P.gen_dev, __ATOMIC_RELAXED, __HIP_MEMORY_SCOPE_AGENT);
        s_gen = g0;
        int d = P.depth_w != nullptr ? 0 : RVM_TEAMS_MAX;
        if (P.depth_w != nullptr) {
            unsigned long long v[RVM_DEPTH_WINDOW];
#pragma unroll
            for (int i = 0; i < RVM_DEPTH_WINDOW; i++)
                v[i] = __hip_atomic_load(P.depth_w + (g0 + 1 + i) % (RVM_DEPTH_WINDOW + 1), __ATOMIC_RELAXED,
                                         __HIP_MEMORY_SCOPE_AGENT);
#pragma unroll
            for (int i = 0; i < RVM_DEPTH_WINDOW; i++)
                if ((v[i] >> 8) < g0 && (v[i] >> 8) + RVM_DEPTH_WINDOW >= g0 && (int)(v[i] & 0xFF) > d)
                    d = (int)(v[i] & 0xFF);
        }
        s_depth = d;
#if RVM_REFINE_RELAXED_COUNT
        asm volatile("s_waitcnt vmcnt(0)" ::: "memory");
        const int done = __hip_atomic_fetch_add(P.rq_n + 3, 1, __ATOMIC_RELAXED, __HIP_MEMORY_SCOPE_AGENT);
#else
        const int done = __hip_atomic_fetch_add(P.rq_n + 3, 1, __ATOMIC_ACQ_REL, __HIP_MEMORY_SCOPE_AGENT);
#endif
        if (done == (int)gridDim.x - 1) {
            for (int i = 0; i < 4; i++) __hip_atomic_store(P.rq_n + i, 0, __ATOMIC_RELAXED, __HIP_MEMORY_SCOPE_AGENT);
            if (!eager && !hedge) __hip_atomic_store(P.gen_dev, g0 + 1, __ATOMIC_RELAXED, __HIP_MEMORY_SCOPE_AGENT);
        }
    }
    __syncthreads();
    RPROF_T(pt_lists);
    const unsigned long long gen = s_gen;
    const int nq[3] = {s_n[0], s_n[1], s_n[2]};
    const int depth_hint = s_depth;
    const int gq0 = (nq[0] + WPB - 1) / WPB, gq1 = (nq[1] + WPB - 1) / WPB, gq2 = (nq[2] + WPB - 1) / WPB;
    const int ng = gq0 + gq1 + gq2;
    const int ntask_split = 2 * gq0 + gq1 + gq2;
    const int gfit = hedge && P.n_cu - hedge < (int)gridDim.x ? P.n_cu - hedge : (int)gridDim.x;
    auto leave = [&]() {
        if (hedge && threadIdx.x == 0) {
            gu64* hw = (gu64*)P.hw;
            if (__hip_atomic_fetch_add(hw + 1, 1ull, __ATOMIC_RELAXED, __HIP_MEMORY_SCOPE_AGENT) + 1 == gridDim.x) {
                __hip_atomic_store(hw + 1, 0ull, __ATOMIC_RELAXED, __HIP_MEMORY_SCOPE_AGENT);
                __hip_atomic_store(hw, (gen << 8) | 1ull, __ATOMIC_RELAXED, __HIP_MEMORY_SCOPE_AGENT);
            }
        }
    };
    const bool split = !eager && P.rq_x != nullptr && gq0 <= P.rq_xgroups && ((int)gridDim.x & 1) == 0 &&
                       ntask_split <= gfit;
    int nteam = 0;
    if (split && P.rq_t != nullptr && P.rvp != nullptr && P.rvp2 != nullptr && rv_out == nullptr &&
        ng <= P.rq_xgroups) {
        nteam = P.n_teams < P.rmax ? P.n_teams : P.rmax;
        if (nteam > (depth_hint > 2 ? depth_hint : 2)) nteam = depth_hint > 2 ? depth_hint : 2;
        while (nteam >= 2 && nteam * ntask_split > gfit) nteam--;
    }
    const bool team = nteam >= 2;
    const int ntask_team = nteam * ntask_split;
    const int ngw = (W + WPB - 1) / WPB;
    const bool esplit = eager && P.eager_split && P.rq_x != nullptr && ngw <= P.rq_xgroups &&
                        ((int)gridDim.x & 1) == 0 && 2 * ngw <= (int)gridDim.x;
    const int ntask = eager ? (esplit ? 2 * ngw : ngw) : (team ? ntask_team : (split ? ntask_split : ng));
    if ((int)blockIdx.x >= ntask) {
        if constexpr (HM) {
            if (hedge && P.hedge_mark && blockIdx.x == gridDim.x - 1 && wv == 0)
                hedge_mark_unneeded(P.rq_w, P.rq_cap, P.htab, P.hw, nq[0], nq[1], nq[2], gen, hedge, WPB);
        }
        leave();
        return;
    }

    extern __shared__ double s_sched[];
    __shared__ double s_rv[2][2][RVM_MAX_LEVELS][64];
    __shared__ int s_enc[2][RVM_MAX_LEVELS][64];
    __shared__ double s_init[8][64];
    __shared__ double s_chi[2][64], s_lb[2][64];
    __shared__ double s_pest[2][64], s_best[2][64], s_bchi[2][64];
    __shared__ int s_open[2][64];
    __shared__ int s_live[64];
    __shared__ int s_stw[64];
    __shared__ double s_lpw[64];
    __shared__ double s_acc[3][64];
    __shared__ int s_dmode[64];
    __shared__ unsigned long long s_mask[2];
    __shared__ int s_xfault;
    __shared__ double s_tc2[2][64], s_te2[2][64];
    __shared__ int s_ter[2][64];
    __shared__ int s_cancel[2];
    __shared__ int s_eitems[64], s_eli[64], s_eany;
    __shared__ int s_emask;
    __shared__ int s_hix[2][64];
    __shared__ int s_skip[64];
    const int emax = P.fwd.n_epochs > P.bwd.n_epochs ? P.fwd.n_epochs : P.bwd.n_epochs;
    for (int dd = 0; dd < 2; dd++) {
        const DirSched& SD = dd ? P.bwd : P.fwd;
        double* b = s_sched + (size_t)dd * 4 * emax;
        const int ED = SD.n_epochs;
        int* bn = reinterpret_cast<int*>(b + 3 * ED);
        for (int i = threadIdx.x; i < ED; i += blockDim.x) {
            b[i] = SD.seg_h1[i];
            b[ED + i] = SD.obs_rv[i];
            b[2 * ED + i] = SD.obs_s2[i];
            bn[i] = SD.seg_n[i];
            bn[ED + i] = SD.obs_idx[i];
        }
    }
    RPROF_T(pt_sched);
    const bool stretch = sa.c != nullptr;
    const bool mh = sa.mh_scale != nullptr;
    const bool mapped = stretch || mh || sa.fd_x != nullptr;

    for (int t = blockIdx.x; t < ntask; t += gridDim.x) {
        int g = t, own = -1, tm = 0;
        if (team) {
            if (t < 2 * nteam * gq0) {
                g = t / (2 * nteam);
                const int r = t - g * 2 * nteam;
                own = r & 1;
                tm = r >> 1;
            } else {
                const int u = t - 2 * nteam * gq0;
                g = gq0 + u / nteam;
                tm = u - (u / nteam) * nteam;
            }
        } else if (esplit) {
            g = t >> 1;
            own = t & 1;
        } else if (split) {
            if (t < 2 * gq0) {
                g = t >> 1;
                own = t & 1;
            } else {
                g = t - gq0;
            }
        }
        int li = g < gq0 ? 0 : (g < gq0 + gq1 ? 1 : 2);
        const int base = (li == 0 ? g : (li == 1 ? g - gq0 : g - gq0 - gq1)) * WPB;
        int cnt = nq[li] - base < WPB ? nq[li] - base : WPB;
        const int* items = P.rq_w + (size_t)li * P.rq_cap + base;
        gu64* ef = eager ? (gu64*)(P.eflag + (size_t)g * RVM_EFLAG_WORDS) : nullptr;
        if (eager) {
            const int w0 = g * WPB;
            __syncthreads();
            if (threadIdx.x < 64) {
                s_eitems[threadIdx.x] = w0 + (int)threadIdx.x < W ? w0 + (int)threadIdx.x : w0;
                s_eli[threadIdx.x] = -1;
            }
            if (threadIdx.x == 0) s_eany = 0;
            __syncthreads();
            for (int l2 = 0; l2 < 3; l2++)
                for (int i = threadIdx.x; i < nq[l2]; i += blockDim.x) {
                    const int wl = P.rq_w[(size_t)l2 * P.rq_cap + i];
                    if (wl >= w0 && wl < w0 + WPB) {
                        s_eli[wl - w0] = l2;
                        s_eany = 1;
                    }
                }
            __syncthreads();
            if (!s_eany) {
                if (threadIdx.x == 0)
                    __hip_atomic_store(ef, (gen << 8) | 1ull, __ATOMIC_RELAXED, __HIP_MEMORY_SCOPE_AGENT);
                continue;
            }
            items = s_eitems;
            cnt = WPB;
        }
        const int wo = items[slot < cnt ? slot : 0];
        int kind = 0, wk = wo, jst = 0, jp = 0;
        double zst = 0.0, zp = 0.0;
        if (stretch) stretch_slot(sa, wo, kind, wk, zst, jst, zp, jp);
#ifdef RVM_PROFILE
        asm volatile("s_waitcnt vmcnt(0) lgkmcnt(0)" ::: "memory");
#endif
        RPROF_T(pt_slot);
        double rowv[R];
#pragma unroll
        for (int r = 0; r < R; r++) rowv[r] = walker_param(mapped, params, W, wk, sa, r, zst, jst, kind, zp, jp);
#ifdef RVM_PROFILE
        asm volatile("s_waitcnt vmcnt(0) lgkmcnt(0)" ::: "memory");
#endif
        RPROF_T(pt_rows);
        Lane<NP> s;
        int status = RVM_STATUS_OK;
        double e2w;
        walker_setup<NP, D3, L>(rowv, pl_idx, hill_factor, s, status, e2w);
        RPROF_T(pt_setup);
        __syncthreads();
        if (wv == 0) {
            s_init[0][lane] = s.rx;
            s_init[1][lane] = s.ry;
            s_init[2][lane] = s.vx;
            s_init[3][lane] = s.vy;
            s_init[4][lane] = s.rz;
            s_init[5][lane] = s.vz;
            s_init[6][lane] = s.r;
            s_init[7][lane] = s.ir;
            if (lane < WPB) {
                const int lli = eager ? s_eli[lane] : li;
                int skip = 0;
                if (P.skip_variants && stretch && sa.n_spec > 0 && sa.dec != nullptr && lane < cnt && lli >= 0) {
                    int k2 = 0, wk2 = 0, j2 = 0, jp2 = 0;
                    double z2 = 0.0, zp2 = 0.0;
                    stretch_slot(sa, items[lane], k2, wk2, z2, j2, zp2, jp2);
                    const long long jl = (long long)j2 - sa.s0_begin;
                    if (k2 != 0 && jl >= 0 && jl < sa.n_spec && P.rq_mark[jl] != (int32_t)gen)
                        skip = (k2 == 2) != (sa.dec[jl] == 1);
                }
                s_skip[lane] = skip;
                const bool v = lane < cnt && lli >= 0 && !skip;
                const int wl = items[lane < cnt ? lane : 0];
                const bool of = v && lli != 2, ob = v && lli != 1;
                s_open[0][lane] = of ? 1 : 0;
                s_open[1][lane] = ob ? 1 : 0;
                s_chi[0][lane] = of ? 0.0 : P.rq_c[wl];
                s_chi[1][lane] = ob ? 0.0 : P.rq_c[(size_t)P.rq_cap + wl];
                s_lb[0][lane] = s_chi[0][lane];
                s_lb[1][lane] = s_chi[1][lane];
                for (int d2i = 0; d2i < 2; d2i++) {
                    s_pest[d2i][lane] = INFINITY;
                    s_best[d2i][lane] = INFINITY;
                    s_bchi[d2i][lane] = 0.0;
                }
                s_live[lane] = v ? 1 : 0;
                s_stw[lane] = RVM_STATUS_NONFINITE;
                s_lpw[lane] = -INFINITY;
            }
            const int lli = lane < WPB ? (eager ? s_eli[lane] : li) : -1;
            const bool live0 = lane < WPB && lane < cnt && lli >= 0 && !s_skip[lane < WPB ? lane : 0];
            const uint64_t m0 = ballot(live0 && lli != 2);
            const uint64_t m1 = ballot(live0 && lli != 1);
            if (lane == 0) {
                s_mask[0] = m0;
                s_mask[1] = m1;
                s_xfault = 0;
                s_cancel[0] = s_cancel[1] = 0;
            }
        }
        const int wme = items[lane < WPB && lane < cnt ? lane : 0];
        if (wv == 0 && lane < WPB) {
            int dmode = 0;
            double dz = 0.0, du = 0.0, dl = 0.0;
            if (lane < cnt && (!eager || s_eli[lane] >= 0) && P.ext_mult > 0 && P.cut)
                accept_inputs(sa, wme, dmode, dz, du, dl);
            s_dmode[lane] = dmode;
            s_acc[0][lane] = dz;
            s_acc[1][lane] = du;
            s_acc[2][lane] = dl;
        }
        __syncthreads();

        const size_t ks = (size_t)(P.n_teams - 1);
        gu64* tpub = team && tm < nteam - 1 ? (gu64*)(P.rq_t + ((size_t)g * ks + tm) * 16 * 64) : nullptr;
        gu64* tflag = team && tm < nteam - 1 ? (gu64*)(P.rq_tf + (size_t)g * P.n_teams + tm) : nullptr;
        gu64* tprev = team && tm > 0 ? (gu64*)(P.rq_t + ((size_t)g * ks + tm - 1) * 16 * 64) : nullptr;
        gu64* tpflag = team && tm > 0 ? (gu64*)(P.rq_tf + (size_t)g * P.n_teams + tm - 1) : nullptr;
        gu64* tdone = team ? (gu64*)(P.rq_tf + (size_t)g * P.n_teams + ks) : nullptr;
        const size_t plane2 = (size_t)2 * P.lvx_emax * P.lvx_stride;
        bool cancelled = false;
        auto pass_eval = [&](DirState& q, const int rfp, const double c2, const double e2, const double d2,
                             const int er) __attribute__((always_inline)) -> bool {
            const bool fin = isfinite(c2) && isfinite(e2);
            if (!er && !fin) {
                q.open = 3;
                return false;
            }
            const double en = e2 / P.npoints;
            const bool stall = fin && rfp >= 2 && !(en < 0.5 * q.pest);
            if (fin && en < q.best) {
                q.best = en;
                q.bchi = c2;
            }
            q.pest = fin ? en : INFINITY;
            if (er) {
                q.open = 2;
            } else if (fin && !(en > P.rtol_dir)) {
                q.open = 0;
                q.chi = c2;
                q.lb = c2;
            } else if (stall && q.best <= RVM_FLOOR_BOUND * P.rtol_dir) {
                q.open = 0;
                q.chi = q.bchi;
                q.lb = q.bchi;
                return true;
            } else {
                q.chi = fin ? c2 : __builtin_nan("");
                q.lb = fin ? open_lb(c2, d2, e2) : 0.0;
            }
            return false;
        };
        auto dir_load = [&](const int dd) __attribute__((always_inline)) {
            return DirState{s_open[dd][lane], s_chi[dd][lane], s_lb[dd][lane], s_pest[dd][lane], s_best[dd][lane],
                            s_bchi[dd][lane]};
        };
        auto dir_store = [&](const int dd, const DirState& q, const bool floor) __attribute__((always_inline)) {
            s_open[dd][lane] = q.open;
            s_chi[dd][lane] = q.chi;
            s_lb[dd][lane] = q.lb;
            s_pest[dd][lane] = q.pest;
            s_best[dd][lane] = q.best;
            s_bchi[dd][lane] = q.bchi;
            if (floor) __hip_atomic_fetch_add(P.counters + 5, 1ull, __ATOMIC_RELAXED, __HIP_MEMORY_SCOPE_AGENT);
        };
        auto pass_result = [&](const int dd, const int rfp, const double c2, const double e2, const double d2,
                               const int er) __attribute__((always_inline)) {
            DirState q = dir_load(dd);
            const bool floor = pass_eval(q, rfp, c2, e2, d2, er);
            dir_store(dd, q, floor);
        };
        auto decide = [&](const DirState& qf, const DirState& qb, const int rfd, int& stw, double& lp,
                          int& ncut) __attribute__((always_inline)) -> bool {
            const int of = qf.open, ob = qb.open;
            stw = RVM_STATUS_OK;
            lp = 0.0;
            ncut = 0;
            if (s_xfault) {
                stw = RVM_STATUS_NONFINITE;
            } else if (of >= 2 || ob >= 2) {
                stw = (of >= 2 ? of : ob) == 2 ? RVM_STATUS_ENCOUNTER : RVM_STATUS_NONFINITE;
            } else if (of == 0 && ob == 0) {
                lp = -((qb.chi + qf.chi) / P.npoints);
                if (!isfinite(lp)) stw = RVM_STATUS_NONFINITE;
            } else {
                const double lp_hi = -((qb.lb + qf.lb) / P.npoints);
                const int dmode = s_dmode[lane];
                if (dmode != 0 && isfinite(lp_hi) &&
                    !accepts_at(sa, dmode, s_acc[0][lane], s_acc[1][lane], s_acc[2][lane], lp_hi)) {
                    lp = lp_hi;
                    ncut = (of ? 1 : 0) + (ob ? 1 : 0);
                } else if (rfd == P.rmax) {
                    stw = RVM_STATUS_UNRESOLVED;
                } else {
                    return false;
// ... 573 lines not shown
                    if (lane < WPB) {
                        auto st = [&](int row, unsigned long long v) {
                            __hip_atomic_store(tpub + row * 64 + lane, v, __ATOMIC_RELAXED, __HIP_MEMORY_SCOPE_AGENT);
                        };
                        auto bits = [](double v) { return (unsigned long long)__double_as_longlong(v); };
                        st(0, (unsigned long long)s_live[lane]);
                        st(1, (unsigned long long)(unsigned)s_stw[lane]);
                        st(2, bits(s_lpw[lane]));
                        for (int d3 = 0; d3 < 2; d3++) {
                            st(3 + 6 * d3, (unsigned long long)(unsigned)s_open[d3][lane]);
                            st(4 + 6 * d3, bits(s_chi[d3][lane]));
                            st(5 + 6 * d3, bits(s_lb[d3][lane]));
                            st(6 + 6 * d3, bits(s_pest[d3][lane]));
                            st(7 + 6 * d3, bits(s_best[d3][lane]));
                            st(8 + 6 * d3, bits(s_bchi[d3][lane]));
                        }
                    }
                    asm volatile("s_waitcnt vmcnt(0)" ::: "memory");
                    if (lane == 0) {
                        __hip_atomic_store(tflag, (gen << 8) | ((m0 | m1) == 0 ? 2ull : 1ull), __ATOMIC_RELAXED,
                                           __HIP_MEMORY_SCOPE_AGENT);
                        if ((m0 | m1) == 0)
                            __hip_atomic_store(tdone, (gen << 8) | 2ull, __ATOMIC_RELAXED, __HIP_MEMORY_SCOPE_AGENT);
                    }
                }
            }
            __syncthreads();
            if (team && tm < nteam - 1) {
                finisher = own <= 0 && (s_mask[0] | s_mask[1]) == 0;
                break;
            }
        }
        RPROF_T(pt_loop1);
        RPROF_RT(prt_loop1);
        if (team && tm == nteam - 1) finisher = own <= 0 && !cancelled;
        if (team && cancelled && tm < nteam - 1 && own <= 0 && threadIdx.x == 0)
            __hip_atomic_store(tflag, (gen << 8) | 2ull, __ATOMIC_RELAXED, __HIP_MEMORY_SCOPE_AGENT);
        if (finisher && threadIdx.x == 0 && P.depth_w != nullptr && rf_last > 0)
            __hip_atomic_fetch_max(P.depth_w + gen % (RVM_DEPTH_WINDOW + 1), (gen << 8) | (unsigned long long)rf_last,
                                   __ATOMIC_RELAXED,
                                   __HIP_MEMORY_SCOPE_AGENT);
        if (finisher && wv == 0 && lane < WPB && lane < cnt && s_skip[lane]) {
            logl_out[wme] = -INFINITY;
            status_out[wme] = RVM_STATUS_SKIPPED;
            __hip_atomic_fetch_add(P.counters + 6, 1ull, __ATOMIC_RELAXED, __HIP_MEMORY_SCOPE_AGENT);
        } else if (finisher && wv == 0 && lane < WPB && lane < cnt && (!eager || s_eli[lane] >= 0)) {
            int k2 = 0, wk2 = wme, j2 = 0, jp2 = 0;
            double z2 = 0.0, zp2 = 0.0;
            if (stretch) stretch_slot(sa, wme, k2, wk2, z2, j2, zp2, jp2);
            auto row = [&](int r) { return walker_param(mapped, params, W, wk2, sa, r, z2, j2, k2, zp2, jp2); };
            const double u3 = stretch ? stretch_u3(sa.seed, (uint64_t)(sa.s0_begin + wme), sa.iteration, sa.half)
                                      : (mh ? mh_u(sa.seed, (uint64_t)(sa.s0_begin + wme), sa.iteration) : 0.0);
            const double lnp0 = (stretch && k2 == 0) || mh ? sa.lnp[wme] : 0.0;
            walker_out<R>(P, sa, wme, s_stw[lane], s_lpw[lane], logl_out, status_out, row, z2, u3, lnp0);
        }
        if (eager && threadIdx.x == 0)
            __hip_atomic_store(ef, (gen << 8) | 1ull, __ATOMIC_RELAXED, __HIP_MEMORY_SCOPE_AGENT);
#ifdef RVM_PROFILE
        if (t == (int)blockIdx.x && lane == 0 && (size_t)blockIdx.x * 8 + wv < RVM_RPROF_MAX_WAVES / 2) {
            unsigned long long* o = rvm_rprof + ((size_t)blockIdx.x * 8 + wv) * RVM_RPROF_SLOTS;
            o[0] = prt_entry;
            o[1] = prt_loop0;
            o[2] = prt_loop1;
            o[3] = __builtin_amdgcn_s_memrealtime();
            o[4] = p_seg;
            o[5] = p_epo;
            o[6] = p_steps;
            o[7] = pt_loop0 - pt_entry;
            o[8] = pt_loop1 - pt_loop0;
            o[9] = (unsigned long long)t | ((unsigned long long)tm << 16) | ((unsigned long long)(own + 1) << 20) |
                   ((unsigned long long)(p_lvl + 1) << 24) | ((unsigned long long)(eager ? 1 : 0) << 28);
            o[10] = p_pass;
            o[11] = (unsigned long long)(unsigned)__builtin_amdgcn_s_getreg((31 << 11) | 4);
            o[12] = p_wait;
            o[13] = pt_lists - pt_entry;
            o[14] = pt_sched - pt_entry;
            o[15] = pt_setup - pt_entry;
            o[16] = pt_slot - pt_entry;
            o[17] = pt_rows - pt_entry;
            o[18] = p_look;
            o[19] = p_info;
            o[20] = p_need;
            o[21] = p_barr;
        }
#endif
    }
    leave();
}

template <int NP, bool D3>
__global__ __launch_bounds__(256) void eager_kernel(const DevPlan P, const int W, const double* __restrict__ params,
                                                    const double hill_factor) {
    constexpr int L = LanesPerWalker<NP>::value;
    constexpr int WPB = 64 / L;
    constexpr int PR = D3 ? 7 : 5;
    constexpr int R = PR * NP;
    const int wv = threadIdx.x >> 6;
    const int lane = threadIdx.x & 63;
    const int slot = lane / L;
    const int pl_idx = lane % L;
    const int nl = P.n_levels;
    const int np2 = P.eager_passes == 2;
    const int g = blockIdx.x >> (1 + np2), dd = (blockIdx.x >> np2) & 1, rf = 1 + (np2 & blockIdx.x);
    const DirSched& SR = dd ? P.bwd : P.fwd;
    const int Er = SR.n_epochs;
    __shared__ double s_rv[2][RVM_MAX_LEVELS][64];
    __shared__ int s_enc[RVM_MAX_LEVELS][64];
    __shared__ int s_cancel[2];
    __shared__ unsigned long long s_gen;
    gu64* ef = (gu64*)(P.eflag + (size_t)g * RVM_EFLAG_WORDS);
    if (threadIdx.x == 0) s_gen = __hip_atomic_load(P.gen_dev, __ATOMIC_RELAXED, __HIP_MEMORY_SCOPE_AGENT);
    __syncthreads();
    const unsigned long long gen = s_gen;
    const unsigned long long ctag = (gen << 8) | 1ull;
    auto cancelled_now = [&]() {
        return __hip_atomic_load(ef, __ATOMIC_RELAXED, __HIP_MEMORY_SCOPE_AGENT) == ctag ||
               __hip_atomic_load(ef + 6 + dd, __ATOMIC_RELAXED, __HIP_MEMORY_SCOPE_AGENT) == ctag;
    };
    gu64* item = ef + 2 + 2 * (rf - 1) + dd;
    if (threadIdx.x == 0) s_cancel[0] = cancelled_now() || !claim_item(item, gen, 1ull);
    __syncthreads();
    if (s_cancel[0]) return;
    const int w0 = g * WPB;
    const int wo = w0 + slot < W ? w0 + slot : w0;
    double rowv[R];
#pragma unroll
    for (int r = 0; r < R; r++) rowv[r] = params[(size_t)r * W + wo];
    Lane<NP> s;
    int status = RVM_STATUS_OK;
    double e2w;
    walker_setup<NP, D3, L>(rowv, pl_idx, hill_factor, s, status, e2w);
    int k = wv < nl ? wv : -1;
    k = __builtin_amdgcn_readfirstlane(k);
    const int k_u = k < 0 ? 0 : k;
    const bool work = k >= 0;
    KickPrep<NP> kq{};
    if (work && Er > 0) kq = kick_prep<NP, L, D3>(s, 1.875);
    const int m_r = P.mult[k_u] << rf;
    const int nt_r = P.nt[k_u];
    const bool late = P.late_mult > 0 && m_r >= P.late_mult;
    const double sc = ldexp(P.inv_mult[k_u], -rf);
    const bool cmb = work && k == 0 && lane < WPB && w0 + lane < W;
    const size_t plane = (size_t)P.lvx_emax * P.lvx_stride;
    gu64* rvo = (gu64*)(P.rve + ((size_t)(rf - 1) * 2 + dd) * plane + (cmb ? w0 + lane : 0));
    double c2 = 0.0, e2 = 0.0;
    bool cancelled = false;
    for (int e = 0; e < Er; e++) {
        const int ns = __builtin_amdgcn_readfirstlane(work ? SR.seg_n[e] * m_r : 0);
        if (ns > 0) segment_gated<D3, NP, L, RVM_REFINE_GUESS>(s, kq, SR.seg_h1[e] * sc, ns, nt_r, late);
        if (work) {
            const double v0 = star_vx<NP, L>(s);
            if (pl_idx == 0) s_rv[e & 1][k_u][slot] = v0;
        }
        if (wv == 0 && lane == 0) s_cancel[e & 1] = cancelled_now();
        __syncthreads();
        if (s_cancel[e & 1]) {
            cancelled = true;
            break;
        }
        if (cmb) {
            double rvx = 0.0, rv3 = 0.0;
            for (int q = 0; q < nl; q++) rvx += P.lw[q] * s_rv[e & 1][q][lane];
            for (int q = 1; q < nl; q++) rv3 += P.lw3[q] * s_rv[e & 1][q][lane];
            const double ob = SR.obs_rv[e], s2 = SR.obs_s2[e];
            const double r = rvx - ob;
            c2 += (r * r) / s2;
// ... 482 lines not shown
```

rvel-mcmc_amd/csrc/rvm_walker.h:

```cpp
#pragma once
#include "rvm_device.h"
#include "rvm_internal.h"
#include "rvm_stretch.h"

#ifndef RVM_DRIFT_ACC
#define RVM_DRIFT_ACC 0
#endif

namespace rvm {

template <int NT, bool GATED, bool D3, int NP, int L, int KG = 0, int ACC = RVM_DRIFT_ACC>
__device__ __forceinline__ void segment_steps(Lane<NP>& s, KickPrep<NP>& kp, double h, int ns, bool& bad) {
    lane_set_step(s, h);
    const VConsts vk = vconsts_for<NT>();
    kick_apply<NP, true, D3>(s, kp);
    int j = 0;
    for (; j + 2 <= ns - 1; j += 2) {
        drift<NT, GATED, D3, NP, KG, ACC>(s, h, bad, vk);
        kp = kick_prep<NP, L, D3>(s, vk.c1875);
        kick_apply<NP, false, D3>(s, kp);
        drift<NT, GATED, D3, NP, KG, ACC>(s, h, bad, vk);
        kp = kick_prep<NP, L, D3>(s, vk.c1875);
        kick_apply<NP, false, D3>(s, kp);
    }
// ... 125 lines not shown
            ph[p] = 0.0;
            pk[p] = 0.0;
            pl[p] = 0.0;
            pix[p] = 0.0;
            piy[p] = 0.0;
        }
    }
    s.p = pl_idx < NP ? pl_idx : NP - 1;
    s.q = pl_idx;
    double Mi[NP + 1];
    Mi[0] = 1.0;
    double hill = 0.0;
#pragma unroll
    for (int p = 0; p < NP; p++) {
        Mi[p + 1] = Mi[p] + s.m[p];
        const double rh = pa[p] * cbrt(s.m[p] / 3.0);
        hill = rh > hill ? rh : hill;
    }
#pragma unroll
    for (int p = 0; p <= NP; p++) s.iMi[p] = 1.0 / Mi[p];
#pragma unroll
    for (int p = 0; p < NP; p++) s.mu[p] = s.m[p] / Mi[p + 1];
    s.dmin2 = (hill_factor * hill) * (hill_factor * hill);
    double own_m = s.m[0], own_a = pa[0], own_h = ph[0], own_k = pk[0], own_l = pl[0], own_M = Mi[1];
    double own_ix = pix[0], own_iy = piy[0];
#pragma unroll
    for (int p = 1; p < NP; p++) {
        if (s.p == p) {
            own_m = s.m[p];
            own_a = pa[p];
            own_h = ph[p];
            own_k = pk[p];
            own_l = pl[p];
            own_M = Mi[p + 1];
            own_ix = pix[p];
            own_iy = piy[p];
        }
    }
    s.GM = own_M;
    double X, Y, VX, VY, Z = 0.0, VZ = 0.0;
    pal_to_cart(1.0 + own_m, own_a, own_l, own_k, own_h, X, Y, VX, VY);
    if constexpr (D3) {
        if (own_ix != 0.0 || own_iy != 0.0) pal_incline(own_ix, own_iy, X, Y, Z, VX, VY, VZ);
    }
    {
        double sx = 0.0, sy = 0.0, sz = 0.0, svx = 0.0, svy = 0.0, svz = 0.0;
        double jx = X, jy = Y, jz = Z, jvx = VX, jvy = VY, jvz = VZ;
#pragma unroll
        for (int q = 0; q < NP - 1; q++) {
            const double xq = grp_get<L>(X, q), yq = grp_get<L>(Y, q);
            const double vxq = grp_get<L>(VX, q), vyq = grp_get<L>(VY, q);
            sx += s.m[q] * xq;
            sy += s.m[q] * yq;
            svx += s.m[q] * vxq;
            svy += s.m[q] * vyq;
            if constexpr (D3) {
                sz += s.m[q] * grp_get<L>(Z, q);
                svz += s.m[q] * grp_get<L>(VZ, q);
            }
            if (s.p == q + 1) {
                jx = X - sx * s.iMi[q + 1];
                jy = Y - sy * s.iMi[q + 1];
                jvx = VX - svx * s.iMi[q + 1];
                jvy = VY - svy * s.iMi[q + 1];
                if constexpr (D3) {
                    jz = Z - sz * s.iMi[q + 1];
                    jvz = VZ - svz * s.iMi[q + 1];
                }
            }
        }
        s.rx = jx;
        s.ry = jy;
        s.vx = jvx;
        s.vy = jvy;
        s.rz = D3 ? jz : 0.0;
        s.vz = D3 ? jvz : 0.0;
    }
    s.r = D3 ? sqrt(s.rx * s.rx + s.ry * s.ry + s.rz * s.rz) : sqrt(s.rx * s.rx + s.ry * s.ry);
    s.ir = 1.0 / s.r;
    s.encm = 0;
    lane_finish(s);
}

typedef __attribute__((address_space(1))) unsigned long long gu64;
typedef __attribute__((address_space(1))) int gi32;
struct SpinClock {
    unsigned long long last;
    __device__ __forceinline__ void restart() { last = __builtin_amdgcn_s_memrealtime(); }
    __device__ __forceinline__ bool expired(unsigned long long ticks) const {
        return __builtin_amdgcn_s_memrealtime() - last > ticks;
    }
};

template <int NT, bool D3, int NP, int L, int KG, int CH = 64, int ACC = RVM_DRIFT_ACC>
__device__ __forceinline__ bool segment_steps_c(Lane<NP>& s, KickPrep<NP>& kp, double h, int ns, const gu64* c0,
                                                const gu64* c1, unsigned long long tag) {
    bool bad = false;
    lane_set_step(s, h);
    const VConsts vk = vconsts_for<NT>();
    kick_apply<NP, true, D3>(s, kp);
    const gu64* w1 = c1 ? c1 : c0;
    auto load = [](const gu64* c) { return __hip_atomic_load(c, __ATOMIC_RELAXED, __HIP_MEMORY_SCOPE_AGENT); };
    int left = ns - 1;
    while (left >= 2) {
        const unsigned long long a = load(c0), b = load(w1);
        const int c = left < CH ? (left & ~1) : CH;
        for (int j = 0; j < c; j += 2) {
            drift<NT, true, D3, NP, KG, ACC>(s, h, bad, vk);
            kp = kick_prep<NP, L, D3>(s, vk.c1875);
            kick_apply<NP, false, D3>(s, kp);
            drift<NT, true, D3, NP, KG, ACC>(s, h, bad, vk);
            kp = kick_prep<NP, L, D3>(s, vk.c1875);
            kick_apply<NP, false, D3>(s, kp);
        }
        left -= c;
        if (__builtin_amdgcn_readfirstlane((int)((a == tag) | (b == tag)))) return false;
    }
    if (left == 1) {
        drift<NT, true, D3, NP, KG, ACC>(s, h, bad, vk);
        kp = kick_prep<NP, L, D3>(s, vk.c1875);
        kick_apply<NP, false, D3>(s, kp);
    }
    drift<NT, true, D3, NP, KG, ACC>(s, h, bad, vk);
    kp = kick_prep<NP, L, D3>(s, vk.c1875);
    kick_apply<NP, true, D3>(s, kp);
    return true;
}

template <bool D3, int NP, int L, int KG = 0, int ACC = RVM_DRIFT_ACC>
__device__ __forceinline__ bool segment_gated_c(Lane<NP>& s, KickPrep<NP>& kp, double h, int ns, int nt,
                                                const gu64* c0, const gu64* c1, unsigned long long tag,
                                                bool late = false) {
    if (late) {
        if (nt <= 6) return segment_steps_c<6, D3, NP, L, KG, 64, 3>(s, kp, h, ns, c0, c1, tag);
        if (nt == 7) return segment_steps_c<7, D3, NP, L, KG, 64, 3>(s, kp, h, ns, c0, c1, tag);
        return segment_steps_c<8, D3, NP, L, KG, 64, 3>(s, kp, h, ns, c0, c1, tag);
    }
    if (nt <= 6) return segment_steps_c<6, D3, NP, L, KG, 64, ACC>(s, kp, h, ns, c0, c1, tag);
    if (nt == 7) return segment_steps_c<7, D3, NP, L, KG, 64, ACC>(s, kp, h, ns, c0, c1, tag);
    return segment_steps_c<8, D3, NP, L, KG, 64, ACC>(s, kp, h, ns, c0, c1, tag);
}

#define RVM_SLOT_EMPTY 0x7FF4DEADBEEF0001ULL
#define RVM_SLOT_STATUS 0xFFF8000000000000ULL
__device__ __forceinline__ unsigned long long slot_status(int st) {
    return RVM_SLOT_STATUS | (unsigned long long)(unsigned)st;
}
__device__ __forceinline__ bool slot_is_status(unsigned long long b) { return (b & 0xFFFFFFFFFFFFFF00ULL) == RVM_SLOT_STATUS; }

#define RVM_ENC_UNRESOLVED 4
#define RVM_ENC_FAULT 8

__device__ __forceinline__ int dir_status(int enc, bool open, double chi2) {
    int st = (enc & 2) ? RVM_STATUS_PRIOR : RVM_STATUS_OK;
    if (st == RVM_STATUS_OK && (enc & 1)) st = RVM_STATUS_ENCOUNTER;
    if (st == RVM_STATUS_OK && (enc & RVM_ENC_FAULT)) st = RVM_STATUS_NONFINITE;
    if (st == RVM_STATUS_OK && (enc & RVM_ENC_UNRESOLVED)) st = RVM_STATUS_UNRESOLVED;
    if (st == RVM_STATUS_OK && !open && !isfinite(chi2)) st = RVM_STATUS_NONFINITE;
    return st;
}

__device__ __forceinline__ double open_lb(double chi2, double d, double est_raw) {
    const double b = chi2 - fmin(d, RVM_CUT_EST_FACTOR * est_raw);
    return b > 0.0 ? b : 0.0;
}

// ... 62 lines not shown
```

rvel-mcmc_amd/rvmcmc/_lib.py:

```python
from __future__ import annotations

import ctypes as C
import os

_HERE = os.path.dirname(os.path.abspath(__file__))
LIB_PATH = os.environ.get("RVM_LIB_PATH") or os.path.join(_HERE, "librvmcmc.so")

RVM_STATUS_OK = 0
RVM_STATUS_PRIOR = 1
RVM_STATUS_ENCOUNTER = 2
RVM_STATUS_NONFINITE = 3
RVM_STATUS_UNRESOLVED = 4
RVM_STATUS_SKIPPED = 5
RVM_MAX_PLANETS = 4
RVM_MAX_LEVELS = 6
RVM_N_COUNTERS = 7
ABI_VERSION = 12


class RvmConfig(C.Structure):
    _fields_ = [
        ("n_planets", C.c_int32),
        ("dt", C.c_double),
        ("n_levels", C.c_int32),
        ("npoints_norm", C.c_double),
        ("level_mult", C.c_int32 * RVM_MAX_LEVELS),
        ("period_hint", C.c_double),
        ("inclined", C.c_int32),
        ("resolve_tol", C.c_double),
        ("resolve_max", C.c_int32),
    ]


RVM_SMALA_MAX_PARAMS = 20
RVM_MAX_PARAM_ROWS = 7 * RVM_MAX_PLANETS


class ParamMapC(C.Structure):
    _fields_ = [
        ("n_rows", C.c_int32),
        ("src", C.c_int32 * RVM_MAX_PARAM_ROWS),
        ("base", C.c_double * RVM_MAX_PARAM_ROWS),
    ]


class SmalaCache(C.Structure):
    _fields_ = [(k, C.c_void_p) for k in ("lp", "grad", "mu", "L", "G", "logdet", "ok")]


class RvmError(RuntimeError):
    pass


_dp = C.c_void_p
SIGNATURES = {
    "rvm_abi_version": (C.c_int, []),
    "rvm_smala_derive": (C.c_int, [C.c_int32, C.c_int32, C.c_int32, _dp, C.c_double, _dp, _dp, _dp, _dp, _dp,
                                   C.c_double, C.c_double, C.c_double, C.POINTER(SmalaCache), _dp]),
    "rvm_smala_metric": (C.c_int, [C.c_int32, C.c_int32, _dp, _dp, _dp, _dp, _dp, C.c_double, C.c_double,
                                   C.POINTER(SmalaCache), _dp]),
    "rvm_smala_propose": (C.c_int, [C.c_int32, C.c_int32, C.c_int64, _dp, C.POINTER(SmalaCache), C.c_double,
                                    C.c_uint64, C.c_uint64, _dp, _dp, _dp]),
    "rvm_smala_accept": (C.c_int, [C.c_int32, C.c_int32, C.c_int64, _dp, C.POINTER(SmalaCache), _dp,
                                   C.POINTER(SmalaCache), C.c_double, C.c_uint64, C.c_uint64, _dp, _dp, _dp, _dp]),
    "rvm_smala_stencil_logl": (C.c_int, [C.c_void_p, C.POINTER(ParamMapC), C.c_int32, C.c_int32, _dp, C.c_double,
                                         _dp, C.c_double, _dp, _dp, _dp, _dp]),
    "rvm_smala_derive_accept": (C.c_int, [C.c_int32, C.c_int32, C.c_int64, C.c_int32, _dp, _dp, C.c_double, _dp, _dp,
                                          _dp, _dp, _dp, C.c_double, C.c_double, C.c_double, C.POINTER(SmalaCache),
                                          C.POINTER(SmalaCache), C.c_uint64, C.c_uint64, _dp, _dp, _dp, _dp]),
    "rvm_smala_derive_sides": (C.c_int, [C.c_int32, C.c_int32, C.c_int32, _dp, C.c_double, _dp, _dp, _dp, _dp, _dp,
                                         C.c_double, C.c_double, C.c_double, C.POINTER(SmalaCache), _dp]),
    "rvm_smala_center_accept": (C.c_int, [C.c_int32, C.c_int32, C.c_int64, _dp, _dp, _dp, _dp, C.POINTER(SmalaCache),
                                          C.POINTER(SmalaCache), C.c_double, C.c_uint64, C.c_uint64, _dp, _dp, _dp,
                                          _dp]),
    "rvm_smala_metric_accept": (C.c_int, [C.c_int32, C.c_int32, C.c_int64, _dp, _dp, _dp, _dp, _dp, _dp, C.c_double,
                                          C.c_double, C.POINTER(SmalaCache), C.POINTER(SmalaCache), C.c_uint64,
                                          C.c_uint64, _dp, _dp, _dp, _dp]),
    "rvm_last_error": (C.c_char_p, []),
    "rvm_plan_create": (C.c_int, [C.POINTER(RvmConfig), C.POINTER(C.c_double), C.POINTER(C.c_double),
                                  C.POINTER(C.c_double), C.c_int32, C.c_int32, C.POINTER(C.c_void_p)]),
    "rvm_plan_destroy": (None, [C.c_void_p]),
    "rvm_plan_faults": (C.c_int, [C.c_void_p, C.c_int32, C.POINTER(C.c_int64), C.POINTER(C.c_int64),
                                  C.POINTER(C.c_int64), C.POINTER(C.c_int64), C.POINTER(C.c_int64), _dp]),
    "rvm_plan_set_handoff_timeout": (C.c_int, [C.c_void_p, C.c_double]),
    "rvm_plan_time_kernels": (C.c_int, [C.c_void_p, C.c_int32]),
    "rvm_plan_kernel_times": (C.c_int, [C.c_void_p, C.POINTER(C.c_float), C.POINTER(C.c_float), C.c_int32,
                                        C.POINTER(C.c_int32)]),
    "rvm_plan_extension": (C.c_int, [C.c_void_p, C.POINTER(C.c_int32)]),
    "rvm_plan_set_verify_eccentricity": (C.c_int, [C.c_void_p, C.c_double]),
    "rvm_plan_set_certain_reject": (C.c_int, [C.c_void_p, C.c_int32]),
    "rvm_plan_counters": (C.c_int, [C.c_void_p, C.c_int32, C.POINTER(C.c_int64), C.c_int32, C.c_void_p]),
    "rvm_plan_hedge_stats": (C.c_int, [C.c_void_p, C.c_int32, C.POINTER(C.c_int64), C.POINTER(C.c_int64),
                                       C.POINTER(C.c_int64), C.c_void_p]),
    "rvm_plan_hedge_marks": (C.c_int, [C.c_void_p, C.c_int32, C.POINTER(C.c_int64), C.POINTER(C.c_int64), C.c_void_p]),
    "rvm_plan_hedge_waits": (C.c_int, [C.c_void_p, C.c_int32, C.POINTER(C.c_int64), C.POINTER(C.c_int64),
                                       C.POINTER(C.c_int64), C.c_void_p]),
    "rvm_plan_info": (C.c_int, [C.c_void_p, C.POINTER(C.c_int32), C.POINTER(C.c_int32), C.POINTER(C.c_int32),
                                C.POINTER(C.c_int32)]),
    "rvm_logl_batch": (C.c_int, [C.c_void_p, C.c_int32, _dp, C.c_double, _dp, _dp, _dp, _dp]),
    "rvm_stretch_propose": (C.c_int, [C.c_int32, C.c_int32, C.c_int64, _dp, C.c_int32, _dp, C.c_double, C.c_uint64,
                                      C.c_uint64, C.c_uint32, _dp, _dp, _dp, _dp]),
    "rvm_stretch_accept": (C.c_int, [C.c_int32, C.c_int32, C.c_int64, _dp, _dp, _dp, _dp, _dp, C.c_uint64, C.c_uint64,
                                     C.c_uint32, _dp, _dp, _dp]),
    "rvm_pt_stretch_propose": (C.c_int, [C.c_int32, C.c_int32, C.c_int32, _dp, _dp, C.c_double, C.c_uint64,
                                         C.c_uint64, C.c_uint32, _dp, _dp, _dp, _dp]),
    "rvm_pt_stretch_accept": (C.c_int, [C.c_int32, C.c_int32, C.c_int32, _dp, _dp, _dp, _dp, _dp, _dp, C.c_uint64,
                                        C.c_uint64, C.c_uint32, _dp, _dp, _dp]),
    "rvm_pt_swap": (C.c_int, [C.c_int32, C.c_int32, C.c_int32, _dp, _dp, _dp, _dp, _dp, C.c_uint64, C.c_uint64, _dp,
                              _dp, _dp]),
    "rvm_pt_ladder_update": (C.c_int, [C.c_int32, C.c_int32, _dp, _dp, _dp, C.c_double, _dp, _dp, _dp, _dp, _dp, _dp,
                                       _dp]),
    "rvm_stretch_half_step": (C.c_int, [C.c_void_p, C.POINTER(ParamMapC), C.c_int32, C.c_int32, C.c_int64, _dp, _dp,
                                        _dp, C.c_int32, _dp, C.c_double, C.c_uint64, C.c_uint64, C.c_uint32,
                                        C.c_double, _dp, _dp, _dp, _dp]),
    "rvm_stretch_iteration_begin": (C.c_int, [C.c_void_p, C.POINTER(ParamMapC), C.c_int32, C.c_int32, C.c_int64,
                                              C.c_int64, _dp, _dp, _dp, _dp, C.c_int32, _dp, _dp, C.c_double, C.c_uint64,
                                              C.c_uint64, C.c_double, _dp, _dp, _dp, _dp, _dp]),
    "rvm_stretch_iteration_end": (C.c_int, [C.c_int32, C.c_int32, C.c_int64, C.c_int64, _dp, _dp, _dp, _dp, _dp,
                                            _dp, _dp, C.c_int32, _dp, _dp, _dp, _dp, C.c_double, C.c_uint64,
                                            C.c_uint64, _dp, _dp, _dp, _dp]),
    "rvm_mh_propose": (C.c_int, [C.c_int32, C.c_int32, C.c_int64, _dp, _dp, C.c_double, C.c_uint64, C.c_uint64, _dp,
                                 _dp, _dp]),
    "rvm_mh_accept": (C.c_int, [C.c_int32, C.c_int32, C.c_int64, _dp, _dp, _dp, _dp, C.c_uint64, C.c_uint64, _dp, _dp,
                                _dp]),
    "rvm_mh_step": (C.c_int, [C.c_void_p, C.POINTER(ParamMapC), C.c_int32, C.c_int32, C.c_int64, _dp, _dp, _dp,
                              C.c_double, C.c_uint64, C.c_uint64, C.c_double, _dp, _dp, _dp, _dp]),
    "rvm_chain_record": (C.c_int, [C.c_int32, C.c_int32, _dp, C.c_int64, C.c_int64, C.c_int64, _dp, C.c_int64,
                                   C.c_int64, _dp, _dp, _dp]),
    "rvm_chain_moments": (C.c_int, [_dp, C.c_int32, C.c_int32, C.c_int64, C.c_int64, _dp, _dp, _dp]),
    "rvm_chain_autocov_workspace_bytes": (C.c_size_t, [C.c_int32, C.c_int32, C.c_int32]),
    "rvm_chain_autocov": (C.c_int, [_dp, _dp, C.c_int32, C.c_int32, C.c_int64, C.c_int64, C.c_int32, C.c_int32, _dp,
                                    _dp, _dp]),
    "rvm_fd_params": (C.c_int, [C.c_int32, C.c_int32, _dp, C.c_double, _dp, _dp, _dp]),
    "rvm_logl_derivs_workspace_bytes": (C.c_size_t, [C.c_int32, C.c_int32]),
    "rvm_logl_derivs": (C.c_int, [C.c_void_p, C.c_int32, _dp, C.c_int32, C.POINTER(C.c_int32), C.c_double, _dp, _dp,
                                  _dp, _dp, _dp, _dp]),
}

_lib = None


def load():
    global _lib
    if _lib is not None:
        return _lib
    if not os.path.exists(LIB_PATH):
        raise RvmError(
            f"librvmcmc.so not found at {LIB_PATH}: build it with `make -C rvel-mcmc_amd` "
            "(or __graft_entry__.build()); there is no CPU fallback")
    try:
        lib = C.CDLL(LIB_PATH)
    except OSError as e:
        raise RvmError(f"failed to load {LIB_PATH}: {e}") from e
    for name, (res, args) in SIGNATURES.items():
        fn = getattr(lib, name)
        fn.restype = res
        fn.argtypes = args
    if lib.rvm_abi_version() != ABI_VERSION:
        raise RvmError("librvmcmc.so ABI version mismatch")
    _lib = lib
    return lib


def check(rc: int, what: str):
    if rc != 0:
        msg = load().rvm_last_error()
        raise RvmError(f"{what} failed ({rc}): {msg.decode() if msg else ''}")


def stream_handle(stream=None) -> int:
    import torch

    s = stream if stream is not None else torch.cuda.current_stream()
    return int(s.cuda_stream)
```

rvel-mcmc_amd/rvmcmc/engine.py:

```python
from __future__ import annotations

import ctypes as C
import math
from dataclasses import dataclass
from typing import Optional

import numpy as np

from . import _lib

KERNEL_KEYS = ("m", "a", "h", "k", "l")
KERNEL_KEYS_INCLINED = KERNEL_KEYS + ("ix", "iy")
SUPPORTED_KEYS = set(KERNEL_KEYS_INCLINED)


def level_multipliers(levels) -> tuple:
    if isinstance(levels, (int, np.integer)):
        mult = tuple(range(1, int(levels) + 1))
    else:
        mult = tuple(int(m) for m in levels)
    if not 1 <= len(mult) <= _lib.RVM_MAX_LEVELS:
        raise ValueError(f"1..{_lib.RVM_MAX_LEVELS} Richardson levels supported, got {len(mult)}")
    if len(set(mult)) != len(mult) or min(mult) < 1 or max(mult) > 64:
        raise ValueError("level multipliers must be distinct integers in 1..64")
# ... 73 lines not shown


def default_device():
    torch = _torch()
    if not torch.cuda.is_available():
        raise _lib.RvmError("no HIP device visible: the likelihood runs only on the GPU (no CPU fallback)")
    return torch.device("cuda", torch.cuda.current_device())


class LoglPlan:

    def __init__(self, t, rv, sigma, npoints, n_planets, dt, levels=4, max_walkers=4096, device=None,
                 period_hint=0.0, inclined=False, resolve=(0.0, 0)):
        torch = _torch()
        self.lib = _lib.load()
        self.device = torch.device(device) if device is not None else default_device()
        t = np.ascontiguousarray(np.asarray(t, dtype=np.float64))
        rv = np.ascontiguousarray(np.asarray(rv, dtype=np.float64))
        sigma = np.ascontiguousarray(np.asarray(sigma, dtype=np.float64))
        if not (len(t) == len(rv) == len(sigma)):
            raise ValueError("t, rv and sigma must have the same length")
        self.n_obs = len(t)
        self.n_planets = int(n_planets)
        self.dt = float(dt)
        self.mult = level_multipliers(levels)
        self.n_levels = len(self.mult)
        self.period_hint = float(period_hint)
        self.inclined = bool(inclined)
        self.rows = (7 if self.inclined else 5) * self.n_planets
        self.npoints = float(npoints)
        self.max_walkers = int(max_walkers)
        self.resolve_tol, self.resolve_max = float(resolve[0]), int(resolve[1])
        self.ecc_guard = float(resolve[2]) if len(resolve) > 2 else 0.0
        self.certain_reject = bool(resolve[3]) if len(resolve) > 3 else True
        lm = (C.c_int32 * _lib.RVM_MAX_LEVELS)(*self.mult)
        cfg = _lib.RvmConfig(self.n_planets, self.dt, self.n_levels, self.npoints, lm, self.period_hint,
                             int(self.inclined), self.resolve_tol, self.resolve_max)
        handle = C.c_void_p()
        dp = C.POINTER(C.c_double)
        with torch.cuda.device(self.device):
            rc = self.lib.rvm_plan_create(C.byref(cfg), t.ctypes.data_as(dp), rv.ctypes.data_as(dp),
                                          sigma.ctypes.data_as(dp), self.n_obs, self.max_walkers, C.byref(handle))
        _lib.check(rc, "rvm_plan_create")
        self._h = handle
        ext = C.c_int32()
        _lib.check(self.lib.rvm_plan_extension(self._h, C.byref(ext)), "rvm_plan_extension")
        self.ext_mult = ext.value
        if self.ecc_guard > 0.0:
            _lib.check(self.lib.rvm_plan_set_verify_eccentricity(self._h, self.ecc_guard),
                       "rvm_plan_set_verify_eccentricity")
        if not self.certain_reject:
            _lib.check(self.lib.rvm_plan_set_certain_reject(self._h, 0), "rvm_plan_set_certain_reject")

    def faults(self, reset=False, stream=None) -> dict:
        vals = (C.c_int64 * _lib.RVM_N_COUNTERS)()
        _lib.check(self.lib.rvm_plan_counters(self._h, int(bool(reset)), vals, _lib.RVM_N_COUNTERS,
                                              _lib.stream_handle(stream)), "rvm_plan_counters")
        f = dict(handoff_timeouts=vals[0], nonfinite=vals[1], unresolved=vals[2], refined=vals[3],
                 truncated=vals[4], floor_settled=vals[5], skipped=vals[6])
        if reset:
            tot = self.__dict__.setdefault("totals", dict.fromkeys(f, 0))
            for k, v in f.items():
                tot[k] += v
        return f

    def hedge_stats(self, reset=False, stream=None) -> dict:
        h, r, m = C.c_int64(), C.c_int64(), C.c_int64()
        _lib.check(self.lib.rvm_plan_hedge_stats(self._h, int(bool(reset)), C.byref(h), C.byref(r), C.byref(m),
                                                 _lib.stream_handle(stream)), "rvm_plan_hedge_stats")
        return dict(hedged=h.value, replayed=r.value, missed=m.value)

    def hedge_marks(self, reset=False, stream=None) -> dict:
        m, g = C.c_int64(), C.c_int64()
        _lib.check(self.lib.rvm_plan_hedge_marks(self._h, int(bool(reset)), C.byref(m), C.byref(g),
                                                 _lib.stream_handle(stream)), "rvm_plan_hedge_marks")
        return dict(marked=m.value, gave_up=g.value)

    def hedge_waits(self, reset=False, stream=None) -> dict:
        w, h, g = C.c_int64(), C.c_int64(), C.c_int64()
        _lib.check(self.lib.rvm_plan_hedge_waits(self._h, int(bool(reset)), C.byref(w), C.byref(h), C.byref(g),
                                                 _lib.stream_handle(stream)), "rvm_plan_hedge_waits")
        return dict(waited=w.value, late_hits=h.value, gave_way=g.value)

    def check_faults(self, what="plan", stream=None, group=None) -> dict:
        f = self.faults(reset=True, stream=stream)
        bad = [f["handoff_timeouts"], f["nonfinite"], f["unresolved"] if self.resolve_max > 0 else 0]
        if group is not None:
            torch = _torch()
            dist = torch.distributed
            dev = self.device if dist.get_backend(group) == "nccl" else torch.device("cpu")
            t = torch.tensor(bad, dtype=torch.int64, device=dev)
            dist.all_reduce(t, group=group)
            bad = [int(v) for v in t.cpu()]
        if any(bad):
            raise _lib.RvmError(f"{what}: {bad[0]} level-split hand-off timeout(s), {bad[1]} non-finite "
                                f"log-likelihood(s), {bad[2]} walker(s) not resolved to the plan's tolerance after "
                                f"{self.resolve_max} halvings on the GPU (rvm_plan_faults"
                                f"{', summed over the ranks' if group is not None else ''})")
        return f

    def time_kernels(self, max_launches):
        _lib.check(self.lib.rvm_plan_time_kernels(self._h, int(max_launches)), "rvm_plan_time_kernels")

    def kernel_times(self, max_launches=4096):
        a = (C.c_float * max_launches)()
        b = (C.c_float * max_launches)()
        n = C.c_int32()
        _lib.check(self.lib.rvm_plan_kernel_times(self._h, a, b, int(max_launches), C.byref(n)), "rvm_plan_kernel_times")
        return np.array(a[:n.value], dtype=np.float64), np.array(b[:n.value], dtype=np.float64)

    def set_handoff_timeout(self, seconds):
        _lib.check(self.lib.rvm_plan_set_handoff_timeout(self._h, float(seconds)), "rvm_plan_set_handoff_timeout")

    def info(self):
        vals = [C.c_int32() for _ in range(4)]
        _lib.check(self.lib.rvm_plan_info(self._h, *[C.byref(v) for v in vals]), "rvm_plan_info")
        return dict(steps_fwd=vals[0].value, steps_bwd=vals[1].value, epochs_fwd=vals[2].value,
                    epochs_bwd=vals[3].value)

    def logl(self, params, hill_factor=1.0, want_rv=False, out=None, status=None, rv_out=None, stream=None):
        torch = _torch()
        if params.dtype != torch.float64 or params.device != self.device or params.dim() != 2:
            raise ValueError("params must be a 2-D float64 tensor on the plan's device")
        if params.shape[0] != self.rows:
            raise ValueError(f"params must have {self.rows} rows (m,a,h,k,l{',ix,iy' if self.inclined else ''} "
                             f"per planet)")
        params = params.contiguous()
        W = params.shape[1]
        if W > self.max_walkers:
            raise ValueError(f"{W} walkers exceed the plan's max_walkers={self.max_walkers}")
        if out is None:
            out = torch.empty(W, dtype=torch.float64, device=self.device)
        if status is None:
            status = torch.empty(W, dtype=torch.int32, device=self.device)
        rvp = 0
        if want_rv:
            if rv_out is None:
                rv_out = torch.empty((self.n_obs, W), dtype=torch.float64, device=self.device)
            rvp = rv_out.data_ptr()
        with torch.cuda.device(self.device):
            rc = self.lib.rvm_logl_batch(self._h, W, params.data_ptr(), float(hill_factor), out.data_ptr(),
                                         status.data_ptr(), rvp, _lib.stream_handle(stream))
        _lib.check(rc, "rvm_logl_batch")
        return out, status, (rv_out if want_rv else None)

    def derivs(self, params, dir_rows, hill_factor=1.0, stream=None):
        torch = _torch()
        if params.dtype != torch.float64 or params.device != self.device or params.dim() != 2:
            raise ValueError("params must be a 2-D float64 tensor on the plan's device")
        if params.shape[0] != self.rows:
            raise ValueError(f"params must have {self.rows} rows")
        params = params.contiguous()
        C_ = params.shape[1]
        rows = np.ascontiguousarray(np.asarray(dir_rows, dtype=np.int32))
        P = len(rows)
        f64 = dict(dtype=torch.float64, device=self.device)
        lp = torch.empty(C_, **f64)
        grad = torch.empty((P, C_), **f64)
        hess = torch.empty((P, P, C_), **f64)
        st = torch.empty(C_, dtype=torch.int32, device=self.device)
        nb = int(self.lib.rvm_logl_derivs_workspace_bytes(C_, P))
        ws = torch.empty(max(nb, 8), dtype=torch.uint8, device=self.device)
        with torch.cuda.device(self.device):
            rc = self.lib.rvm_logl_derivs(self._h, C_, params.data_ptr(), P, rows.ctypes.data_as(C.POINTER(C.c_int32)),
                                          float(hill_factor), lp.data_ptr(), grad.data_ptr(), hess.data_ptr(),
                                          st.data_ptr(), ws.data_ptr(), _lib.stream_handle(stream))
# ... 206 lines not shown
```

Measured before the change: 3.214 million.

## Hand walker setup state from logL kernel to refine kernel via per-walker records

When the decision kernel queues a walker for refinement, it now writes a per-walker record holding the initial orbital state, masses, acceptance inputs and stretch metadata, tagged with the current generation. The refine kernel reads that record, when the tags match, instead of recomputing the stretch proposal, the parameter rows and walker_setup. This is meant to cut redundant setup work in the refine path. In exchange it adds global-memory writes in the logL kernel, a larger rq buffer and extra atomics for counters. A new env knob (on by default) and a stats API expose it.

```diff
diff --git a/include/rvmcmc.h b/include/rvmcmc.h
--- a/include/rvmcmc.h
+++ b/include/rvmcmc.h
@@ -57,6 +57,8 @@
 int rvm_plan_hedge_marks(rvm_plan* plan, int32_t reset, int64_t* marked, int64_t* gave_up, void* stream);
 int rvm_plan_hedge_waits(rvm_plan* plan, int32_t reset, int64_t* waited, int64_t* late_hits, int64_t* gave_way,
                          void* stream);
+int rvm_plan_handon(rvm_plan* plan, int32_t reset, int64_t* records_written, int64_t* tasks_from_records,
+                    int64_t* fell_back, int64_t* listed, void* stream);
 int rvm_plan_time_kernels(rvm_plan* plan, int32_t max_launches);
 int rvm_plan_kernel_times(rvm_plan* plan, float* logl_ms, float* refine_ms, int32_t max, int32_t* n_out);
 int rvm_plan_set_handoff_timeout(rvm_plan* plan, double seconds);
diff --git a/rvel-mcmc_amd/csrc/host_sanitize.cpp b/rvel-mcmc_amd/csrc/host_sanitize.cpp
--- a/rvel-mcmc_amd/csrc/host_sanitize.cpp
+++ b/rvel-mcmc_amd/csrc/host_sanitize.cpp
@@ -46,7 +46,7 @@
 static const char* const kKnobNames[] = {
     "RVM_SKIP_VARIANTS", "RVM_LATE_SPO",   "RVM_NO_LEVEL_SPLIT", "RVM_REFINE_TEAMS", "RVM_EAGER_SPLIT",
     "RVM_NO_EXTENSION",  "RVM_REFINE_SPLIT", "RVM_TEAMS_HINT",   "RVM_EAGER",        "RVM_EAGER_PASSES",
-    "RVM_HEDGE",         "RVM_HEDGE_GROUPS", "RVM_HEDGE_MARK",   "RVM_HEDGE_WAIT",
+    "RVM_HEDGE",         "RVM_HEDGE_GROUPS", "RVM_HEDGE_MARK",   "RVM_HEDGE_WAIT",   "RVM_HANDON",
     "RVM_LS_F0"};
 
 static rvm::PlanKnobs knobs_with(const char* name, const char* value) {
@@ -65,7 +65,7 @@
     expect(K.skip_variants == 1 && K.late_spo == 96.0 && !K.no_level_split && K.n_teams == RVM_TEAMS_DEFAULT &&
                K.eager_split == 1 && !K.no_extension && K.refine_split && K.teams_hint && K.eager &&
                K.eager_passes == 1 && K.hedge_groups == RVM_HEDGE_GROUPS_MAX && K.hedge_mark == 1 &&
-               K.hedge_wait == 1,
+               K.hedge_wait == 1 && K.handon == 1,
            "knob defaults");
     expect(knobs_with("RVM_REFINE_TEAMS", "9").n_teams == RVM_TEAMS_MAX, "RVM_REFINE_TEAMS=9 clamps");
     expect(knobs_with("RVM_HEDGE", "0").hedge_groups == 0, "RVM_HEDGE=0");
@@ -75,6 +75,9 @@
     expect(knobs_with("RVM_HEDGE_WAIT", "0").hedge_wait == 0 && knobs_with("RVM_HEDGE_WAIT", "1").hedge_wait == 1 &&
                knobs_with("RVM_HEDGE_WAIT", "2").hedge_wait == 2 && knobs_with("RVM_HEDGE_WAIT", "x").hedge_wait == 1,
            "RVM_HEDGE_WAIT");
+    expect(knobs_with("RVM_HANDON", "0").handon == 0 && knobs_with("RVM_HANDON", "1").handon == 1 &&
+               knobs_with("RVM_HANDON", "x").handon == 1,
+           "RVM_HANDON");
 
     int mult[RVM_MAX_LEVELS] = {}, max_mult = 0;
     expect(check_plan_config(&cfg, t.data(), rv.data(), sg.data(), n_obs, 4096, mult, &max_mult) == nullptr,
@@ -191,9 +194,13 @@
             check_block({{R.x, xg * nt * 256 * 8, true}, {R.xf, xg * nt * 2 * 8, true},
                          {R.t, xg * (nt - 1) * 1024 * 8, true}, {R.tf, xg * nt * 8, true}, {R.tb, xg * 8, true},
                          {R.c, 16 * w, true},
-                         {R.w, 12 * w, false}, {R.n, 16, false}, {R.gen, 8, true}, {R.mark, 4 * w, false},
-                         {R.depth, 8 * (RVM_DEPTH_WINDOW + 1), true}},
+                         {R.w, 12 * w, false}, {R.n, 16, false}, {R.n + 16, 8, true}, {R.gen, 8, true},
+                         {R.hc, 8 * RVM_HANDON_COUNTERS, true}, {R.mark, 4 * w, false},
+                         {R.depth, 8 * (RVM_DEPTH_WINDOW + 1), true}, {R.rec, 8 * RVM_HANDON_DOUBLES * w, true}},
                         R.bytes, "rqmem layout");
+            expect(R.rec == R.mark + handon_offset_from_mark(mw) && R.hc == R.gen + 8 &&
+                       R.hc + 8 * RVM_HANDON_COUNTERS <= R.n + 64,
+                   "hand-on records behind depth_w, counters behind gen_dev");
             expect(R.tb == R.tf + xg * nt * 8, "rq_tb right behind rq_tf");
             expect(R.gen == R.n + 32 && R.mark == R.n + 64 && R.mark % 64 == R.n % 64, "rq_n | gen_dev | rq_mark");
         }
@@ -253,6 +260,9 @@
     int64_t lh = -1;
     expect(rvm_plan_hedge_waits(nullptr, 0, &mk, &lh, &gu, nullptr) < 0 && mk == -1 && lh == -1 && gu == -1,
            "hedge_waits null plan");
+    int64_t nl = -1;
+    expect(rvm_plan_handon(nullptr, 0, &mk, &lh, &gu, &nl, nullptr) < 0 && mk == -1 && lh == -1 && gu == -1 && nl == -1,
+           "handon null plan");
     rvm_param_map pm{};
     expect(rvm_stretch_half_step(nullptr, &pm, 10, 1, 0, nullptr, nullptr, nullptr, 1, nullptr, 2.0, 0, 0, 0, 1.0,
                                  nullptr, nullptr, nullptr, nullptr) < 0,
diff --git a/rvel-mcmc_amd/csrc/rvm_internal.h b/rvel-mcmc_amd/csrc/rvm_internal.h
--- a/rvel-mcmc_amd/csrc/rvm_internal.h
+++ b/rvel-mcmc_amd/csrc/rvm_internal.h
@@ -1,4 +1,5 @@
 #pragma once
+#include <stddef.h>
 #include <stdint.h>
 
 #include "../../include/rvmcmc.h"
@@ -30,6 +31,17 @@
 constexpr int RVM_HW_MARK = RVM_HW_STATS + 3 + 3;
 constexpr int RVM_HW_WAIT = RVM_HW_MARK + 2 * RVM_HEDGE_GROUPS_MAX;
 constexpr int RVM_HW_WORDS = RVM_HW_WAIT + 3;
+constexpr int RVM_HANDON_DOUBLES = 48;
+constexpr int RVM_HANDON_M = 32;
+constexpr int RVM_HANDON_E2W = 36;
+constexpr int RVM_HANDON_DMIN2 = 37;
+constexpr int RVM_HANDON_DZ = 38;
+constexpr int RVM_HANDON_META = 41;
+constexpr int RVM_HANDON_TAG = 42;
+constexpr size_t handon_offset_from_mark(int32_t rq_cap) {
+    return (((size_t)rq_cap * sizeof(int32_t) + 63) & ~(size_t)63) + (RVM_DEPTH_WINDOW + 1) * sizeof(unsigned long long);
+}
+constexpr int RVM_HANDON_COUNTERS = 3;
 
 struct DirSched {
     int32_t n_epochs;
@@ -80,6 +92,7 @@
     unsigned long long* rq_tf;
     double* rvp2;
     int32_t n_teams;
+    int32_t handon;
     unsigned long long* depth_w;
     double* rve;
     double* esum;
@@ -107,6 +120,8 @@
     int32_t lv_emax, lv_stride;
     DirSched fwd, bwd;
 };
+static_assert(sizeof(DevPlan) == 776 && offsetof(DevPlan, handon) == 476 && offsetof(DevPlan, depth_w) == 480,
+              "DevPlan keeps its size and its fields their offsets");
 
 struct StretchArgs {
     const double* c;
diff --git a/rvel-mcmc_amd/csrc/rvm_logl.hip b/rvel-mcmc_amd/csrc/rvm_logl.hip
--- a/rvel-mcmc_amd/csrc/rvm_logl.hip
+++ b/rvel-mcmc_amd/csrc/rvm_logl.hip
@@ -502,6 +502,10 @@
     }
     const int encflag = (int)(((s.encm >> lane) & kick_enc_bits<NP>()) != 0) |
                         (status == RVM_STATUS_PRIOR ? 2 : 0) | (wfault ? RVM_ENC_FAULT : 0);
+    int ho_kind = 0, ho_j = 0;
+    bool ho_listed = false;
+    double* const ho_rec =
+        reinterpret_cast<double*>(reinterpret_cast<char*>(P.rq_mark) + handon_offset_from_mark(P.rq_cap));
     auto finish = [&](const int wo, const double chi2w, const int enc, const bool open, const double lbw, auto&& row,
                       const double z, const double u3, const double lnp0) __attribute__((always_inline)) {
         const int st = dir_status(enc, open, chi2w);
@@ -532,7 +536,7 @@
         const double lp0 = -((cb + cf) / P.npoints);
         if (stw == RVM_STATUS_OK && (of || ob)) {
             int dmode = 0;
-            double dz, du, dl;
+            double dz = 0.0, du = 0.0, dl = 0.0;
             if (P.ext_mult > 0 && P.cut) accept_inputs(sa, wo, dmode, dz, du, dl);
             if (dmode != 0 && isfinite(lp0) && !accepts_at(sa, dmode, dz, du, dl, lp0)) {
                 __hip_atomic_fetch_add(P.counters + 4, (unsigned long long)((of ? 1 : 0) + (ob ? 1 : 0)),
@@ -542,9 +546,24 @@
                 const int ix = __hip_atomic_fetch_add(P.rq_n + li, 1, __ATOMIC_RELAXED, __HIP_MEMORY_SCOPE_AGENT);
                 if (ix < P.rq_cap) {
                     P.rq_w[(size_t)li * P.rq_cap + ix] = wo;
-                    P.rq_mark[wo] = (int32_t)__hip_atomic_load(P.gen_dev, __ATOMIC_RELAXED, __HIP_MEMORY_SCOPE_AGENT);
+                    const unsigned long long g64 = __hip_atomic_load(P.gen_dev, __ATOMIC_RELAXED, __HIP_MEMORY_SCOPE_AGENT);
+                    P.rq_mark[wo] = (int32_t)g64;
                     P.rq_c[wo] = of ? 0.0 : cf;
                     P.rq_c[(size_t)P.rq_cap + wo] = ob ? 0.0 : cb;
+                    if constexpr (DEC) {
+                        if (P.handon) {
+                            double* rec = ho_rec + (size_t)wo * RVM_HANDON_DOUBLES;
+                            unsigned long long* recw = reinterpret_cast<unsigned long long*>(rec);
+                            rec[RVM_HANDON_DZ] = dz;
+                            rec[RVM_HANDON_DZ + 1] = du;
+                            rec[RVM_HANDON_DZ + 2] = dl;
+                            recw[RVM_HANDON_META] = (unsigned long long)(unsigned)dmode |
+                                                    ((unsigned long long)(unsigned)ho_kind << 8) |
+                                                    ((unsigned long long)(unsigned)ho_j << 32);
+                            recw[RVM_HANDON_TAG] = g64;
+                            ho_listed = true;
+                        }
+                    }
                     return;
                 }
                 stw = RVM_STATUS_NONFINITE;
@@ -559,6 +578,8 @@
             double z2, zp2;
             asm volatile("" : "+v"(wo));
             stretch_slot(sa, wo, k2, wk2, z2, j2, zp2, jp2);
+            ho_kind = k2;
+            ho_j = j2;
             auto row = [&](int r) { return walker_param(true, params, W, wk2, sa, r, z2, j2, k2, zp2, jp2); };
             finish(wo, chi2w, enc, open, lbw, row, z2,
                    stretch_u3(sa.seed, (uint64_t)(sa.s0_begin + wo), sa.iteration, sa.half), k2 == 0 ? sa.lnp[wo] : 0.0);
@@ -569,6 +590,30 @@
         } else {
             auto row = [&](int) { return 0.0; };
             finish(w_in, chi2w, enc, open, lbw, row, 0.0, 0.0, 0.0);
+        }
+    };
+
+    auto handon_lanes = [&](const bool by_slot) __attribute__((always_inline)) {
+        if constexpr (DEC) {
+            if (!P.handon) return;
+            const uint64_t lm = ballot(ho_listed);
+            ho_listed = false;
+            if (lm == 0) return;
+            if (valid && ((lm >> (by_slot ? slot : slot * L)) & 1)) {
+                double* rec = ho_rec + (size_t)w * RVM_HANDON_DOUBLES;
+                const double* in = l_init + (size_t)ul * RVM_INIT_DOUBLES + lane;
+#pragma unroll
+                for (int k = 0; k < 8; k++) rec[8 * pl_idx + k] = in[64 * k];
+                if (pl_idx == 0) {
+#pragma unroll
+                    for (int p = 0; p < NP; p++) rec[RVM_HANDON_M + p] = s.m[p];
+                    rec[RVM_HANDON_E2W] = e2w;
+                    rec[RVM_HANDON_DMIN2] = s.dmin2;
+                }
+            }
+            if (lane == 0)
+                __hip_atomic_fetch_add((gu64*)P.gen_dev + 1, (unsigned long long)__builtin_popcountll(lm), __ATOMIC_RELAXED,
+                                       __HIP_MEMORY_SCOPE_AGENT);
         }
     };
 
@@ -1021,6 +1066,7 @@
                 const double lb = cn ? 0.0 : direction_lb(nd, cm, es, (f & 16) != 0 && ((f & 64) == 0 || P.cut_guard_k > 0.0), xc5,
                                                                  (f & 64) != 0 ? P.cut_guard_k * xdd : xdd);
                 if (cl) finish_recompute(w0 + lane, c2, en, nd, lb);
+                handon_lanes(true);
             } else if (valid && pl_idx == 0) {
                 if (lsx && need) {
                     const double* rg = ring + (size_t)(ul * 4 + 2) * RING * WPB + slot;
@@ -1031,6 +1077,7 @@
                                  cenc ? 0.0 : direction_lb(need, chi2m, est, lsx && need0 && (e2w <= P.e2_cut || P.cut_guard_k > 0.0), c5x,
                                                           e2w <= P.e2_cut ? ddx : P.cut_guard_k * ddx));
             }
+            handon_lanes(false);
 #ifdef RVM_PROFILE
             prof_dec(rt_arr, nl - 1);
 #endif
diff --git a/rvel-mcmc_amd/csrc/rvm_plan.hip b/rvel-mcmc_amd/csrc/rvm_plan.hip
--- a/rvel-mcmc_amd/csrc/rvm_plan.hip
+++ b/rvel-mcmc_amd/csrc/rvm_plan.hip
@@ -121,6 +121,7 @@
     P.depth_w = K.teams_hint ? at<unsigned long long>(plan->rqmem, L.depth) : nullptr;
     P.rq_cap = plan->max_walkers;
     P.rq_xgroups = L.xgroups;
+    P.handon = K.handon;
     const unsigned long long gen1 = 1;
     if (hipMemcpy(P.gen_dev, &gen1, sizeof(gen1), hipMemcpyHostToDevice) != hipSuccess) {
         (void)hipGetLastError();
@@ -336,6 +337,28 @@
     return 0;
 }
 
+int rvm_plan_handon(rvm_plan* plan, int32_t reset, int64_t* records_written, int64_t* tasks_from_records,
+                    int64_t* fell_back, int64_t* listed, void* stream) {
+    if (!plan) return fail(-1, "rvm_plan_handon: null plan");
+    unsigned long long h[rvm::RVM_HANDON_COUNTERS] = {}, nl = 0;
+    if (plan->dev.gen_dev != nullptr) {
+        hipStream_t st = (hipStream_t)stream;
+        unsigned long long* d = plan->dev.gen_dev + 1;
+        unsigned long long* dl = reinterpret_cast<unsigned long long*>(plan->dev.rq_n + 4);
+        hipError_t e = hipMemcpyAsync(h, d, sizeof(h), hipMemcpyDeviceToHost, st);
+        if (e == hipSuccess) e = hipMemcpyAsync(&nl, dl, sizeof(nl), hipMemcpyDeviceToHost, st);
+        if (e == hipSuccess && reset) e = hipMemsetAsync(d, 0, sizeof(h), st);
+        if (e == hipSuccess && reset) e = hipMemsetAsync(dl, 0, sizeof(nl), st);
+        if (e == hipSuccess) e = hipStreamSynchronize(st);
+        if (e != hipSuccess) return hip_fail(e, "rvm_plan_handon");
+    }
+    if (records_written) *records_written = (int64_t)h[0];
+    if (tasks_from_records) *tasks_from_records = (int64_t)h[1];
+    if (fell_back) *fell_back = (int64_t)h[2];
+    if (listed) *listed = (int64_t)nl;
+    return 0;
+}
+
 int rvm_plan_faults(rvm_plan* plan, int32_t reset, int64_t* handoff_timeouts, int64_t* nonfinite,
                     int64_t* unresolved, int64_t* refined, int64_t* truncated, void* stream) {
     if (!plan) return fail(-1, "rvm_plan_faults: null plan");
diff --git a/rvel-mcmc_amd/csrc/rvm_plan_host.cpp b/rvel-mcmc_amd/csrc/rvm_plan_host.cpp
--- a/rvel-mcmc_amd/csrc/rvm_plan_host.cpp
+++ b/rvel-mcmc_amd/csrc/rvm_plan_host.cpp
@@ -40,6 +40,7 @@
     K.hedge_mark = starts(getenv("RVM_HEDGE_MARK"), '0') ? 0 : 1;
     const char* hwt = getenv("RVM_HEDGE_WAIT");
     K.hedge_wait = starts(hwt, '0') ? 0 : (starts(hwt, '2') ? 2 : 1);
+    K.handon = starts(getenv("RVM_HANDON"), '0') ? 0 : 1;
     return K;
 }
 
@@ -282,6 +283,8 @@
     L.gen = L.n + 32;
     L.mark = take(L.bytes, ((size_t)max_walkers * sizeof(int32_t) + 63) & ~(size_t)63);
     L.depth = take(L.bytes, (RVM_DEPTH_WINDOW + 1) * u64);
+    L.rec = take(L.bytes, (size_t)max_walkers * RVM_HANDON_DOUBLES * sizeof(double));
+    L.hc = L.gen + u64;
     return L;
 }
 
diff --git a/rvel-mcmc_amd/csrc/rvm_plan_host.h b/rvel-mcmc_amd/csrc/rvm_plan_host.h
--- a/rvel-mcmc_amd/csrc/rvm_plan_host.h
+++ b/rvel-mcmc_amd/csrc/rvm_plan_host.h
@@ -20,6 +20,7 @@
     int32_t hedge_groups;
     int32_t hedge_mark;
     int32_t hedge_wait;
+    int32_t handon;
 };
 PlanKnobs read_plan_knobs();
 
@@ -61,7 +62,7 @@
 };
 XLayout x_layout(size_t nf, size_t nb, int32_t max_walkers, int n_teams);
 struct RqLayout {
-    size_t x, xf, t, tf, tb, c, w, n, gen, mark, depth, bytes;
+    size_t x, xf, t, tf, tb, c, w, n, gen, mark, depth, rec, hc, bytes;
     int32_t xgroups;
 };
 RqLayout rq_layout(int32_t max_walkers, int n_teams);
diff --git a/rvel-mcmc_amd/csrc/rvm_refine_impl.h b/rvel-mcmc_amd/csrc/rvm_refine_impl.h
--- a/rvel-mcmc_amd/csrc/rvm_refine_impl.h
+++ b/rvel-mcmc_amd/csrc/rvm_refine_impl.h
@@ -108,6 +108,18 @@
 };
 
 constexpr int RVM_REFINE_HM = 5;
+template <bool ON, int NP>
+struct HandonRegs {
+    static constexpr bool from_rec = false;
+    static constexpr double acc[3] = {0.0, 0.0, 0.0};
+    static constexpr unsigned long long meta = 0;
+};
+template <int NP>
+struct HandonRegs<true, NP> {
+    bool from_rec = false;
+    double acc[3];
+    unsigned long long meta = 0;
+};
 template <int NP, bool D3, int NW>
 __global__ __launch_bounds__((NW == RVM_REFINE_HM ? 4 : NW) * 64) void refine_kernel(
     const DevPlan P, const int W, const double* __restrict__ params, const double hill_factor,
@@ -158,6 +170,13 @@
         const int done = __hip_atomic_fetch_add(P.rq_n + 3, 1, __ATOMIC_ACQ_REL, __HIP_MEMORY_SCOPE_AGENT);
 #endif
         if (done == (int)gridDim.x - 1) {
+            if constexpr (HM) {
+                if (P.handon) {
+                    unsigned long long nlist = 0;
+                    for (int i = 0; i < 3; i++) nlist += (unsigned long long)(s_n[i] < P.rq_cap ? s_n[i] : P.rq_cap);
+                    __hip_atomic_fetch_add((gu64*)(P.rq_n + 4), nlist, __ATOMIC_RELAXED, __HIP_MEMORY_SCOPE_AGENT);
+                }
+            }
             for (int i = 0; i < 4; i++) __hip_atomic_store(P.rq_n + i, 0, __ATOMIC_RELAXED, __HIP_MEMORY_SCOPE_AGENT);
             if (!eager && !hedge) __hip_atomic_store(P.gen_dev, g0 + 1, __ATOMIC_RELAXED, __HIP_MEMORY_SCOPE_AGENT);
         }
@@ -300,24 +319,66 @@
             cnt = WPB;
         }
         const int wo = items[slot < cnt ? slot : 0];
+        HandonRegs<HM, NP> ho;
+        Lane<NP> s;
+        if constexpr (HM) {
+            if (P.handon && !eager) {
+                const double* recs = reinterpret_cast<const double*>(reinterpret_cast<const char*>(P.rq_mark) +
+                                                                     handon_offset_from_mark(P.rq_cap));
+                const bool inb = wo >= 0 && wo < P.rq_cap;
+                const double* rec = recs + (size_t)(inb ? wo : 0) * RVM_HANDON_DOUBLES;
+                const int wd = items[lane < WPB && lane < cnt ? lane : 0];
+                const bool inbd = wd >= 0 && wd < P.rq_cap;
+                const double* recd = recs + (size_t)(inbd ? wd : 0) * RVM_HANDON_DOUBLES;
+                const unsigned long long tag = reinterpret_cast<const unsigned long long*>(rec)[RVM_HANDON_TAG];
+                const unsigned long long tagd = reinterpret_cast<const unsigned long long*>(recd)[RVM_HANDON_TAG];
+                double v[8], m[NP];
+#pragma unroll
+                for (int k = 0; k < 8; k++) v[k] = rec[8 * pl_idx + k];
+#pragma unroll
+                for (int p = 0; p < NP; p++) m[p] = rec[RVM_HANDON_M + p];
+                const double dmin2 = rec[RVM_HANDON_DMIN2];
+#pragma unroll
+                for (int i = 0; i < 3; i++) ho.acc[i] = recd[RVM_HANDON_DZ + i];
+                ho.meta = reinterpret_cast<const unsigned long long*>(recd)[RVM_HANDON_META];
+                ho.from_rec = ballot(!inb || !inbd || tag != gen || tagd != gen) == 0;
+                if (wv == 0 && lane == 0)
+                    __hip_atomic_fetch_add((gu64*)P.gen_dev + (ho.from_rec ? 2 : 3), 1ull, __ATOMIC_RELAXED,
+                                           __HIP_MEMORY_SCOPE_AGENT);
+                if (ho.from_rec) {
+                    s.rx = v[0];
+                    s.ry = v[1];
+                    s.vx = v[2];
+                    s.vy = v[3];
+                    s.rz = v[4];
+                    s.vz = v[5];
+                    s.r = v[6];
+                    s.ir = v[7];
+#pragma unroll
+                    for (int p = 0; p < NP; p++) s.m[p] = m[p];
+                    lane_consts<NP>(s, pl_idx, dmin2);
+                }
+            }
+        }
         int kind = 0, wk = wo, jst = 0, jp = 0;
         double zst = 0.0, zp = 0.0;
-        if (stretch) stretch_slot(sa, wo, kind, wk, zst, jst, zp, jp);
+        if (stretch && !ho.from_rec) stretch_slot(sa, wo, kind, wk, zst, jst, zp, jp);
 #ifdef RVM_PROFILE
         asm volatile("s_waitcnt vmcnt(0) lgkmcnt(0)" ::: "memory");
 #endif
         RPROF_T(pt_slot);
         double rowv[R];
-#pragma unroll
-        for (int r = 0; r < R; r++) rowv[r] = walker_param(mapped, params, W, wk, sa, r, zst, jst, kind, zp, jp);
+        if (!ho.from_rec) {
+#pragma unroll
+            for (int r = 0; r < R; r++) rowv[r] = walker_param(mapped, params, W, wk, sa, r, zst, jst, kind, zp, jp);
+        }
 #ifdef RVM_PROFILE
         asm volatile("s_waitcnt vmcnt(0) lgkmcnt(0)" ::: "memory");
 #endif
         RPROF_T(pt_rows);
-        Lane<NP> s;
         int status = RVM_STATUS_OK;
         double e2w;
-        walker_setup<NP, D3, L>(rowv, pl_idx, hill_factor, s, status, e2w);
+        if (!ho.from_rec) walker_setup<NP, D3, L>(rowv, pl_idx, hill_factor, s, status, e2w);
         RPROF_T(pt_setup);
         __syncthreads();
         if (wv == 0) {
@@ -335,7 +396,12 @@
                 if (P.skip_variants && stretch && sa.n_spec > 0 && sa.dec != nullptr && lane < cnt && lli >= 0) {
                     int k2 = 0, wk2 = 0, j2 = 0, jp2 = 0;
                     double z2 = 0.0, zp2 = 0.0;
-                    stretch_slot(sa, items[lane], k2, wk2, z2, j2, zp2, jp2);
+                    if (ho.from_rec) {
+                        k2 = (int)((ho.meta >> 8) & 0xFF);
+                        j2 = (int)(ho.meta >> 32);
+                    } else {
+                        stretch_slot(sa, items[lane], k2, wk2, z2, j2, zp2, jp2);
+                    }
                     const long long jl = (long long)j2 - sa.s0_begin;
                     if (k2 != 0 && jl >= 0 && jl < sa.n_spec && P.rq_mark[jl] != (int32_t)gen)
                         skip = (k2 == 2) != (sa.dec[jl] == 1);
@@ -374,14 +440,23 @@
         if (wv == 0 && lane < WPB) {
             int dmode = 0;
             double dz = 0.0, du = 0.0, dl = 0.0;
-            if (lane < cnt && (!eager || s_eli[lane] >= 0) && P.ext_mult > 0 && P.cut)
-                accept_inputs(sa, wme, dmode, dz, du, dl);
+            if (lane < cnt && (!eager || s_eli[lane] >= 0) && P.ext_mult > 0 && P.cut) {
+                if (ho.from_rec) {
+                    dmode = (int)(ho.meta & 0xFF);
+                    dz = ho.acc[0];
+                    du = ho.acc[1];
+                    dl = ho.acc[2];
+                } else {
+                    accept_inputs(sa, wme, dmode, dz, du, dl);
+                }
+            }
             s_dmode[lane] = dmode;
             s_acc[0][lane] = dz;
             s_acc[1][lane] = du;
             s_acc[2][lane] = dl;
         }
         __syncthreads();
+        RPROF_T(pt_acc);
 
         const size_t ks = (size_t)(P.n_teams - 1);
         gu64* tpub = team && tm < nteam - 1 ? (gu64*)(P.rq_t + ((size_t)g * ks + tm) * 16 * 64) : nullptr;
@@ -1121,6 +1196,7 @@
             o[19] = p_info;
             o[20] = p_need;
             o[21] = p_barr;
+            o[22] = pt_acc - pt_entry;
         }
 #endif
     }
diff --git a/rvel-mcmc_amd/csrc/rvm_walker.h b/rvel-mcmc_amd/csrc/rvm_walker.h
--- a/rvel-mcmc_amd/csrc/rvm_walker.h
+++ b/rvel-mcmc_amd/csrc/rvm_walker.h
@@ -231,6 +231,28 @@
     lane_finish(s);
 }
 
+template <int NP>
+__device__ __forceinline__ void lane_consts(Lane<NP>& s, const int pl_idx, const double dmin2) {
+    s.p = pl_idx < NP ? pl_idx : NP - 1;
+    s.q = pl_idx;
+    double Mi[NP + 1];
+    Mi[0] = 1.0;
+#pragma unroll
+    for (int p = 0; p < NP; p++) Mi[p + 1] = Mi[p] + s.m[p];
+#pragma unroll
+    for (int p = 0; p <= NP; p++) s.iMi[p] = 1.0 / Mi[p];
+#pragma unroll
+    for (int p = 0; p < NP; p++) s.mu[p] = s.m[p] / Mi[p + 1];
+    s.dmin2 = dmin2;
+    double own_M = Mi[1];
+#pragma unroll
+    for (int p = 1; p < NP; p++)
+        if (s.p == p) own_M = Mi[p + 1];
+    s.GM = own_M;
+    s.encm = 0;
+    lane_finish(s);
+}
+
 typedef __attribute__((address_space(1))) unsigned long long gu64;
 typedef __attribute__((address_space(1))) int gi32;
 struct SpinClock {
diff --git a/rvel-mcmc_amd/rvmcmc/_lib.py b/rvel-mcmc_amd/rvmcmc/_lib.py
--- a/rvel-mcmc_amd/rvmcmc/_lib.py
+++ b/rvel-mcmc_amd/rvmcmc/_lib.py
@@ -95,6 +95,8 @@
     "rvm_plan_hedge_marks": (C.c_int, [C.c_void_p, C.c_int32, C.POINTER(C.c_int64), C.POINTER(C.c_int64), C.c_void_p]),
     "rvm_plan_hedge_waits": (C.c_int, [C.c_void_p, C.c_int32, C.POINTER(C.c_int64), C.POINTER(C.c_int64),
                                        C.POINTER(C.c_int64), C.c_void_p]),
+    "rvm_plan_handon": (C.c_int, [C.c_void_p, C.c_int32, C.POINTER(C.c_int64), C.POINTER(C.c_int64),
+                                  C.POINTER(C.c_int64), C.POINTER(C.c_int64), C.c_void_p]),
     "rvm_plan_info": (C.c_int, [C.c_void_p, C.POINTER(C.c_int32), C.POINTER(C.c_int32), C.POINTER(C.c_int32),
                                 C.POINTER(C.c_int32)]),
     "rvm_logl_batch": (C.c_int, [C.c_void_p, C.c_int32, _dp, C.c_double, _dp, _dp, _dp, _dp]),
diff --git a/rvel-mcmc_amd/rvmcmc/engine.py b/rvel-mcmc_amd/rvmcmc/engine.py
--- a/rvel-mcmc_amd/rvmcmc/engine.py
+++ b/rvel-mcmc_amd/rvmcmc/engine.py
@@ -179,6 +179,12 @@
                                                  _lib.stream_handle(stream)), "rvm_plan_hedge_waits")
         return dict(waited=w.value, late_hits=h.value, gave_way=g.value)
 
+    def handon(self, reset=False, stream=None) -> dict:
+        w, t, f, n = C.c_int64(), C.c_int64(), C.c_int64(), C.c_int64()
+        _lib.check(self.lib.rvm_plan_handon(self._h, int(bool(reset)), C.byref(w), C.byref(t), C.byref(f), C.byref(n),
+                                            _lib.stream_handle(stream)), "rvm_plan_handon")
+        return dict(records_written=w.value, tasks_from_records=t.value, fell_back=f.value, listed=n.value)
+
     def check_faults(self, what="plan", stream=None, group=None) -> dict:
         f = self.faults(reset=True, stream=stream)
         bad = [f["handoff_timeouts"], f["nonfinite"], f["unresolved"] if self.resolve_max > 0 else 0]
```

New measurement: 3.238 million, median of 6. No clear change (+0.8%).
